# qingstor-incubating/qsfs-fuse

Hardware: AMD Instinct MI355X
Metric: GiB/s MD5-hashed, device-resident 10 MB chunks, batch=512; % HBM-read peak (higher is better)
Workload: dtype u32; 1 GPU; batch=512 x 10 MiB chunks per GPU, device-resident (BASELINE config 2); global_batch=512, chunk_bytes=10485760, parallelism=single GPU, kernel=producer/consumer (qsmd5_batch_pc64_kernel)

## Files before the change

qsfs-fuse_amd/csrc/md5_core.h:

```cpp
#pragma once

#include <hip/hip_runtime.h>
#include <stdint.h>

namespace qsmd5 {

struct Md5Tables {
  static constexpr uint32_t K[64] = {
      0xd76aa478u, 0xe8c7b756u, 0x242070dbu, 0xc1bdceeeu, 0xf57c0fafu, 0x4787c62au,
      0xa8304613u, 0xfd469501u, 0x698098d8u, 0x8b44f7afu, 0xffff5bb1u, 0x895cd7beu,
      0x6b901122u, 0xfd987193u, 0xa679438eu, 0x49b40821u, 0xf61e2562u, 0xc040b340u,
      0x265e5a51u, 0xe9b6c7aau, 0xd62f105du, 0x02441453u, 0xd8a1e681u, 0xe7d3fbc8u,
      0x21e1cde6u, 0xc33707d6u, 0xf4d50d87u, 0x455a14edu, 0xa9e3e905u, 0xfcefa3f8u,
      0x676f02d9u, 0x8d2a4c8au, 0xfffa3942u, 0x8771f681u, 0x6d9d6122u, 0xfde5380cu,
      0xa4beea44u, 0x4bdecfa9u, 0xf6bb4b60u, 0xbebfbc70u, 0x289b7ec6u, 0xeaa127fau,
      0xd4ef3085u, 0x04881d05u, 0xd9d4d039u, 0xe6db99e5u, 0x1fa27cf8u, 0xc4ac5665u,
      0xf4292244u, 0x432aff97u, 0xab9423a7u, 0xfc93a039u, 0x655b59c3u, 0x8f0ccc92u,
      0xffeff47du, 0x85845dd1u, 0x6fa87e4fu, 0xfe2ce6e0u, 0xa3014314u, 0x4e0811a1u,
      0xf7537e82u, 0xbd3af235u, 0x2ad7d2bbu, 0xeb86d391u};
};

constexpr uint32_t kInit0 = 0x67452301u;
constexpr uint32_t kInit1 = 0xefcdab89u;
constexpr uint32_t kInit2 = 0x98badcfeu;
constexpr uint32_t kInit3 = 0x10325476u;

__host__ __device__ constexpr int md5_shift(int i) {
  return (i < 16)   ? ((i & 3) == 0 ? 7 : (i & 3) == 1 ? 12 : (i & 3) == 2 ? 17 : 22)
         : (i < 32) ? ((i & 3) == 0 ? 5 : (i & 3) == 1 ? 9 : (i & 3) == 2 ? 14 : 20)
         : (i < 48) ? ((i & 3) == 0 ? 4 : (i & 3) == 1 ? 11 : (i & 3) == 2 ? 16 : 23)
                    : ((i & 3) == 0 ? 6 : (i & 3) == 1 ? 10 : (i & 3) == 2 ? 15 : 21);
}

__host__ __device__ constexpr int md5_word(int i) {
  return (i < 16) ? i
         : (i < 32) ? ((5 * (i - 16) + 1) & 15)
         : (i < 48) ? ((3 * (i - 32) + 5) & 15)
                    : ((7 * (i - 48)) & 15);
}

__host__ __device__ constexpr uint32_t md5_fn_host(int round, uint32_t x, uint32_t y, uint32_t z) {
  return round == 0   ? ((x & y) | (~x & z))
         : round == 1 ? ((x & z) | (y & ~z))
         : round == 2 ? (x ^ y ^ z)
                      : (y ^ (x | ~z));
}
__host__ __device__ constexpr uint32_t md5_bitop3_imm(int round) {
  return md5_fn_host(round, 0xF0u, 0xCCu, 0xAAu) & 0xFFu;
}

template <int I>
__device__ __forceinline__ uint32_t md5_round_fn(uint32_t b, uint32_t c, uint32_t d) {
  return __builtin_amdgcn_bitop3_b32(b, c, d, md5_bitop3_imm(I >> 4));
}

template <int I>
__device__ __forceinline__ void md5_steps(uint32_t (&v)[4], const uint32_t (&w)[16]) {
  if constexpr (I < 64) {
    constexpr int ia = (4 - (I & 3)) & 3;
    constexpr int ib = (ia + 1) & 3;
    constexpr int ic = (ia + 2) & 3;
    constexpr int id = (ia + 3) & 3;
    const uint32_t amk = v[ia] + w[md5_word(I)] + Md5Tables::K[I];
    const uint32_t t = amk + md5_round_fn<I>(v[ib], v[ic], v[id]);
    v[ia] = v[ib] + __builtin_rotateleft32(t, md5_shift(I));
    md5_steps<I + 1>(v, w);
  }
}

template <int I, int kEnd = 64>
__device__ __forceinline__ void md5_steps_mk(uint32_t (&v)[4], const uint32_t (&mk)[64]) {
  if constexpr (I < kEnd) {
    constexpr int ia = (4 - (I & 3)) & 3;
    constexpr int ib = (ia + 1) & 3;
    constexpr int ic = (ia + 2) & 3;
    constexpr int id = (ia + 3) & 3;
    const uint32_t t = v[ia] + md5_round_fn<I>(v[ib], v[ic], v[id]) + mk[I];
    v[ia] = v[ib] + __builtin_rotateleft32(t, md5_shift(I));
    md5_steps_mk<I + 1, kEnd>(v, mk);
  }
}

__device__ __forceinline__ void md5_compress_mk(uint32_t (&st)[4], const uint32_t (&mk)[64]) {
  uint32_t v[4] = {st[0], st[1], st[2], st[3]};
  md5_steps_mk<0>(v, mk);
  st[0] += v[0];
  st[1] += v[1];
  st[2] += v[2];
  st[3] += v[3];
}

__device__ __forceinline__ void md5_compress(uint32_t (&st)[4], const uint32_t (&w)[16]) {
  uint32_t v[4] = {st[0], st[1], st[2], st[3]};
  md5_steps<0>(v, w);
  st[0] += v[0];
  st[1] += v[1];
  st[2] += v[2];
  st[3] += v[3];
}

typedef uint32_t u32x4 __attribute__((ext_vector_type(4)));
typedef uint32_t u32x4_a4 __attribute__((ext_vector_type(4), aligned(4)));
#define QS_GLOBAL __attribute__((address_space(1)))

template <bool kNT = false>
__device__ __forceinline__ u32x4 load16_a4(const uint32_t* p) {
  if constexpr (kNT)
    return __builtin_nontemporal_load((const QS_GLOBAL u32x4_a4*)(reinterpret_cast<uintptr_t>(p)));
  else
    return *(const QS_GLOBAL u32x4_a4*)(reinterpret_cast<uintptr_t>(p));
}
__device__ __forceinline__ uint32_t load4(const uint32_t* p) {
  return *(const QS_GLOBAL uint32_t*)(reinterpret_cast<uintptr_t>(p));
}

__device__ __forceinline__ void unpack4(uint32_t (&w)[16], int k, u32x4 q) {
  w[4 * k + 0] = q.x;
  w[4 * k + 1] = q.y;
  w[4 * k + 2] = q.z;
  w[4 * k + 3] = q.w;
}

}
```

qsfs-fuse_amd/csrc/md5_kernels.hip:

```cpp
#include <hip/hip_runtime.h>
#include <stdint.h>

#include "md5_core.h"

namespace qsmd5 {

struct ChunkDesc {
  const uint8_t* ptr;
  uint64_t len;
};

__device__ __forceinline__ void blocks_aligned4(uint32_t (&st)[4], const uint32_t* p,
                                                uint32_t nblk) {
  if (nblk == 0) return;
  const uint32_t last = nblk - 1;
  u32x4 a0, a1, a2, a3, b0, b1, b2, b3, c0, c1, c2, c3, d0, d1, d2, d3;
#define QS_LOAD(X, blk)                                   \
  do {                                                    \
    const uint32_t* q_ = p + (uint64_t)(blk) * 16u;       \
    X##0 = load16_a4(q_);                                 \
    X##1 = load16_a4(q_ + 4);                             \
    X##2 = load16_a4(q_ + 8);                             \
    X##3 = load16_a4(q_ + 12);                            \
  } while (0)
#define QS_COMPRESS(X)            \
  do {                            \
    uint32_t w_[16];              \
    unpack4(w_, 0, X##0);         \
    unpack4(w_, 1, X##1);         \
    unpack4(w_, 2, X##2);         \
    unpack4(w_, 3, X##3);         \
    md5_compress(st, w_);         \
  } while (0)
  QS_LOAD(a, 0);
  QS_LOAD(b, min(1u, last));
  QS_LOAD(c, min(2u, last));
  QS_LOAD(d, min(3u, last));
  uint32_t j = 0;
  for (; j + 4 <= nblk; j += 4) {
    QS_COMPRESS(a);
    QS_LOAD(a, min(j + 4, last));
    QS_COMPRESS(b);
    QS_LOAD(b, min(j + 5, last));
    QS_COMPRESS(c);
    QS_LOAD(c, min(j + 6, last));
    QS_COMPRESS(d);
    QS_LOAD(d, min(j + 7, last));
  }
  if (j < nblk) QS_COMPRESS(a);
  if (j + 1 < nblk) QS_COMPRESS(b);
  if (j + 2 < nblk) QS_COMPRESS(c);
#undef QS_COMPRESS
#undef QS_LOAD
}

__device__ __forceinline__ void blocks_unaligned(uint32_t (&st)[4], const uint8_t* bp,
                                                 uint32_t nblk) {
  const uintptr_t a = reinterpret_cast<uintptr_t>(bp);
  const uint32_t* base = reinterpret_cast<const uint32_t*>(a & ~uintptr_t(3));
  const uint32_t off = static_cast<uint32_t>(a & 3u);
  for (uint32_t j = 0; j < nblk; ++j) {
    const uint32_t* q = base + (uint64_t)j * 16u;
    u32x4 x0 = load16_a4(q), x1 = load16_a4(q + 4), x2 = load16_a4(q + 8),
          x3 = load16_a4(q + 12);
    uint32_t e = load4(q + 16);
    uint32_t d[17] = {x0.x, x0.y, x0.z, x0.w, x1.x, x1.y, x1.z, x1.w, x2.x,
                      x2.y, x2.z, x2.w, x3.x, x3.y, x3.z, x3.w, e};
    uint32_t w[16];
#pragma unroll
    for (int k = 0; k < 16; ++k) w[k] = __builtin_amdgcn_alignbyte(d[k + 1], d[k], off);
    md5_compress(st, w);
  }
}

__device__ __forceinline__ void finish(uint32_t (&st)[4], const uint8_t* tp, uint32_t rem,
                                       uint64_t total_len) {
  const uintptr_t a = reinterpret_cast<uintptr_t>(tp);
  const uint32_t* base = reinterpret_cast<const uint32_t*>(a & ~uintptr_t(3));
  const uint32_t off = static_cast<uint32_t>(a & 3u);
  uint32_t d[17];
#pragma unroll
  for (int k = 0; k < 17; ++k)
    d[k] = (rem != 0u && (uint32_t)(4 * k) < off + rem) ? load4(base + k) : 0u;
  uint32_t w[16];
#pragma unroll
  for (int k = 0; k < 16; ++k) {
    uint32_t x = __builtin_amdgcn_alignbyte(d[k + 1], d[k], off);
    const uint32_t lo = 4u * k;
    uint32_t m = rem >= lo + 4u ? 0xffffffffu : rem <= lo ? 0u : ((1u << (8u * (rem - lo))) - 1u);
    x &= m;
    if ((rem >> 2) == (uint32_t)k) x |= 0x80u << (8u * (rem & 3u));
    w[k] = x;
  }
  const uint64_t bits = total_len << 3;
  if (rem < 56u) {
    w[14] = (uint32_t)bits;
    w[15] = (uint32_t)(bits >> 32);
    md5_compress(st, w);
  } else {
    md5_compress(st, w);
#pragma unroll
    for (int k = 0; k < 14; ++k) w[k] = 0u;
    w[14] = (uint32_t)bits;
    w[15] = (uint32_t)(bits >> 32);
    md5_compress(st, w);
  }
}

__device__ __forceinline__ void hash_message(uint32_t (&st)[4], const uint8_t* p, uint64_t len) {
  const uint32_t nblk = (uint32_t)(len >> 6);
  if ((reinterpret_cast<uintptr_t>(p) & 3u) == 0)
    blocks_aligned4(st, reinterpret_cast<const uint32_t*>(p), nblk);
  else
    blocks_unaligned(st, p, nblk);
  finish(st, p + ((uint64_t)nblk << 6), (uint32_t)(len & 63u), len);
}


__device__ __forceinline__ uint32_t wave_max_u32(uint32_t v) {
#pragma unroll
  for (int o = 32; o > 0; o >>= 1) v = max(v, (uint32_t)__shfl_xor((int)v, o, 64));
  return v;
}

__device__ __forceinline__ uint32_t rfl_u32(uint32_t v) {
  return (uint32_t)__builtin_amdgcn_readfirstlane((int)v);
}

__device__ __forceinline__ uint32_t wave_min_u32(uint32_t v) {
#pragma unroll
  for (int o = 32; o > 0; o >>= 1) v = min(v, (uint32_t)__shfl_xor((int)v, o, 64));
  return v;
}

__device__ __forceinline__ void lds_barrier() {
  asm volatile("s_waitcnt lgkmcnt(0)\n\ts_barrier" ::: "memory");
}

constexpr int kPcHalf = 4;
constexpr int kPcLead = 8;
constexpr int kLgkmcnt0 = 0xC07F;

struct PcBlockRegs {
  u32x4 q[4];
  uint32_t e;
};

template <bool kNT>
__device__ __forceinline__ void pc_load_block(PcBlockRegs& r, const uint32_t* base, uint32_t off,
                                              uint32_t blk) {
  const uint32_t* q = base + (uint64_t)blk * 16u;
  r.q[0] = load16_a4<kNT>(q);
  r.q[1] = load16_a4<kNT>(q + 4);
  r.q[2] = load16_a4<kNT>(q + 8);
  r.q[3] = load16_a4<kNT>(q + 12);
  r.e = off ? load4(q + 16) : 0u;
}

__device__ __forceinline__ void pc_write_mk(u32x4 (*slot)[64], uint32_t lane, const PcBlockRegs& r,
                                            uint32_t off) {
  uint32_t d[17] = {r.q[0].x, r.q[0].y, r.q[0].z, r.q[0].w, r.q[1].x, r.q[1].y,
                    r.q[1].z, r.q[1].w, r.q[2].x, r.q[2].y, r.q[2].z, r.q[2].w,
                    r.q[3].x, r.q[3].y, r.q[3].z, r.q[3].w, r.e};
  uint32_t w[16];
#pragma unroll
  for (int k = 0; k < 16; ++k) w[k] = __builtin_amdgcn_alignbyte(d[k + 1], d[k], off);
#pragma unroll
  for (int g = 0; g < 16; ++g) {
    u32x4 m;
    m.x = w[md5_word(4 * g + 0)] + Md5Tables::K[4 * g + 0];
    m.y = w[md5_word(4 * g + 1)] + Md5Tables::K[4 * g + 1];
    m.z = w[md5_word(4 * g + 2)] + Md5Tables::K[4 * g + 2];
    m.w = w[md5_word(4 * g + 3)] + Md5Tables::K[4 * g + 3];
    slot[g][lane] = m;
  }
}


template <bool kAllLive, int kHalf = kPcHalf, int kLead = 0, int kLead2 = 0>
__device__ __forceinline__ void chain_phase(uint32_t (&st)[4], const u32x4 (*ring)[16][64],
                                            uint32_t s0, uint32_t lane, uint32_t blk0,
                                            uint32_t nblk) {
  u32x4 a[16], b[16];
  auto read_slot = [&](u32x4 (&dst)[16], uint32_t slot) {
#pragma unroll
    for (int g = 0; g < 16; ++g) dst[g] = ring[slot][g][lane];
  };
  auto unpack_slot = [&](uint32_t (&mk)[64], const u32x4 (&src)[16]) {
#pragma unroll
    for (int g = 0; g < 16; ++g) {
      mk[4 * g + 0] = src[g].x;
      mk[4 * g + 1] = src[g].y;
      mk[4 * g + 2] = src[g].z;
      mk[4 * g + 3] = src[g].w;
    }
  };
  auto compress_slot = [&](const u32x4 (&src)[16]) {
    uint32_t mk[64];
    unpack_slot(mk, src);
    md5_compress_mk(st, mk);
  };
  read_slot(a, s0);
  if constexpr (kLead > 0) {
    static_assert(kLead % 4 == 0 && kLead < 64, "kLead: whole ds_read_b128 groups");
    __builtin_amdgcn_sched_barrier(0);
    __builtin_amdgcn_s_waitcnt((kLgkmcnt0 & ~(0xF << 8)) | ((16 - kLead / 4) << 8));
    __builtin_amdgcn_sched_barrier(0);
    const bool run0 = kAllLive || blk0 < nblk;
    uint32_t mk[64];
    unpack_slot(mk, a);
    uint32_t v[4] = {st[0], st[1], st[2], st[3]};
    if (run0) md5_steps_mk<0, kLead>(v, mk);
    constexpr int kRest = kLead2 > kLead ? kLead2 : kLead;
    if constexpr (kLead2 > kLead) {
      static_assert(kLead2 % 4 == 0 && kLead2 < 64, "kLead2: whole ds_read_b128 groups");
      __builtin_amdgcn_sched_barrier(0);
      __builtin_amdgcn_s_waitcnt((kLgkmcnt0 & ~(0xF << 8)) | ((16 - kLead2 / 4) << 8));
      __builtin_amdgcn_sched_barrier(0);
      if (run0) md5_steps_mk<kLead, kLead2>(v, mk);
    }
    __builtin_amdgcn_sched_barrier(0);
    __builtin_amdgcn_s_waitcnt(kLgkmcnt0);
    if (1 < kHalf) read_slot(b, s0 + 1);
    __builtin_amdgcn_sched_barrier(0);
    if (run0) {
      md5_steps_mk<kRest, 64>(v, mk);
      st[0] += v[0];
      st[1] += v[1];
      st[2] += v[2];
      st[3] += v[3];
    }
  }
#pragma unroll
  for (int h = (kLead > 0 ? 1 : 0); h < kHalf; ++h) {
    __builtin_amdgcn_sched_barrier(0);
    __builtin_amdgcn_s_waitcnt(kLgkmcnt0);
    if (h + 1 < kHalf) read_slot((h & 1) ? a : b, s0 + h + 1);
    __builtin_amdgcn_sched_barrier(0);
    if (kAllLive || blk0 + (uint32_t)h < nblk) compress_slot((h & 1) ? b : a);
  }
}


}

using namespace qsmd5;

extern "C" __global__ __launch_bounds__(64) void qsmd5_batch_kernel(
    const ChunkDesc* __restrict__ chunks, const uint32_t* __restrict__ order, uint32_t n,
    uint32_t* __restrict__ digests) {
  const uint32_t t = blockIdx.x * 64u + threadIdx.x;
  if (t >= n) return;
  const uint32_t idx = order ? order[t] : t;
  const ChunkDesc cd = chunks[idx];
  uint32_t st[4] = {kInit0, kInit1, kInit2, kInit3};
  hash_message(st, cd.ptr, cd.len);
  u32x4 o = {st[0], st[1], st[2], st[3]};
  *reinterpret_cast<u32x4*>(digests + 4u * (uint64_t)idx) = o;
}

extern "C" __global__ __launch_bounds__(64) void qsmd5_final_kernel(uint32_t* __restrict__ state,
                                                                    const uint8_t* tail,
                                                                    uint32_t rem,
                                                                    uint64_t total_len) {
  if (threadIdx.x != 0 || blockIdx.x != 0) return;
  uint32_t st[4] = {state[0], state[1], state[2], state[3]};
  finish(st, tail, rem, total_len);
  state[0] = st[0];
  state[1] = st[1];
  state[2] = st[2];
  state[3] = st[3];
}

namespace {
constexpr uint32_t kLcgA = 1103515245u;
constexpr uint32_t kLcgC = 12345u;
constexpr uint32_t kSeg = 1024u;

__device__ __forceinline__ uint32_t lcg_jump(uint32_t x, uint64_t n) {
  uint32_t am = kLcgA, cm = kLcgC;
  uint32_t ar = 1u, cr = 0u;
  while (n) {
    if (n & 1u) {
      ar = ar * am;
      cr = cr * am + cm;
    }
    cm = cm * am + cm;
    am = am * am;
    n >>= 1;
  }
  return ar * x + cr;
}
}

extern "C" __global__ __launch_bounds__(256) void qsmd5_lcg_fill_kernel(
    uint8_t* __restrict__ base, uint64_t stride, uint64_t len, uint32_t seed0,
    uint32_t nchunks, uint64_t segs_per_chunk) {
  const uint64_t g = (uint64_t)blockIdx.x * blockDim.x + threadIdx.x;
  const uint64_t chunk = g / segs_per_chunk;
  if (chunk >= nchunks) return;
  const uint64_t seg = g - chunk * segs_per_chunk;
  const uint64_t start = seg * kSeg;
  if (start >= len) return;
  const uint64_t end = start + kSeg < len ? start + kSeg : len;
  uint32_t x = lcg_jump(seed0 + (uint32_t)chunk, start);
  uint8_t* out = base + chunk * stride;
  uint64_t i = start;
  if (((reinterpret_cast<uintptr_t>(out) + start) & 3u) == 0) {
    for (; i + 4 <= end; i += 4) {
      uint32_t v = 0;
#pragma unroll
      for (int b = 0; b < 4; ++b) {
        x = x * kLcgA + kLcgC;
        v |= ((x >> 16) & 0xffu) << (8 * b);
      }
      *reinterpret_cast<uint32_t*>(out + i) = v;
    }
  }
  for (; i < end; ++i) {
    x = x * kLcgA + kLcgC;
    out[i] = (uint8_t)(x >> 16);
  }
}

constexpr uint32_t kSkewMinBlocks = 1u << 19;
template <bool kColumn, int kDepth = 1, int kHalf = kPcHalf, bool kNT = false, bool kTrace = false,
          int kPace = 0, int kGap = 0, int kLead = kPcLead, int kLead2 = 0, int kProbe = 0>
__device__ __forceinline__ void pc_body(const ChunkDesc* __restrict__ chunks,
                                        const uint32_t* __restrict__ order, uint32_t n,
                                        uint32_t* __restrict__ digests, uint64_t col_off,
                                        uint64_t col_w, uint32_t* __restrict__ states,
                                        uint32_t skew, uint64_t* __restrict__ trace = nullptr,
                                        uint32_t lanes = 64) {
  __shared__ u32x4 ring[2 * kHalf][16][64];
  const uint32_t lane = threadIdx.x & 63u;
  const uint32_t wave = threadIdx.x >> 6;
  const uint32_t t = blockIdx.x * lanes + lane;
  const bool live = lane < lanes && t < n;
  uint32_t idx = 0;
  ChunkDesc cd = {nullptr, 0};
  uint64_t seg = 0;
  bool final = true;
  if (live) {
    if (kColumn) {
      idx = order[t];
      cd = chunks[t];
      const uint64_t rest = cd.len - col_off;
      final = rest <= col_w;
      seg = final ? rest : col_w;
    } else {
      idx = order ? order[t] : t;
      cd = chunks[idx];
      seg = cd.len;
    }
  }
  const uint32_t nblk = (uint32_t)(seg >> 6);
  const bool skewed = !kColumn && skew != 0 && wave_max_u32(nblk) >= kSkewMinBlocks;
  const uint32_t delta = (skewed && nblk) ? skew * ((lane * 37u) & 63u) : 0u;
  const uint32_t phases = (wave_max_u32(nblk + delta) + kHalf - 1) / kHalf;
  const uintptr_t pa = reinterpret_cast<uintptr_t>(cd.ptr);
  const uint32_t off = (uint32_t)(pa & 3u);

  if (wave == 1) {
    const uint32_t* base = reinterpret_cast<const uint32_t*>(pa & ~uintptr_t(3));
    const uint32_t last = nblk ? nblk - 1 : 0;
    PcBlockRegs r[kDepth][kHalf];
    if constexpr ((kProbe & 2) != 0) {
#pragma unroll
      for (int k = 0; k < kDepth; ++k)
#pragma unroll
        for (int h = 0; h < kHalf; ++h) r[k][h] = PcBlockRegs{{lane, lane, lane, lane}, lane};
    }
    auto load_phase = [&](PcBlockRegs (&rs)[kHalf], uint32_t p) {
      if constexpr ((kProbe & 2) != 0) return;
      if (nblk) {
#pragma unroll
        for (int h = 0; h < kHalf; ++h) {
          const uint32_t j = p * kHalf + h;
          pc_load_block<kNT>(rs[h], base, off, j < delta ? 0u : min(j - delta, last));
        }
      }
    };
    auto write_phase = [&](const PcBlockRegs (&rs)[kHalf], uint32_t p) {
      if (nblk) {
#pragma unroll
        for (int h = 0; h < kHalf; ++h) {
          if constexpr (kGap > 0) {
            if (h) __builtin_amdgcn_s_sleep(kGap);
          }
          if constexpr ((kProbe & 1) == 0) pc_write_mk(ring[(p & 1u) * kHalf + h], lane, rs[h], off);
        }
      }
    };
    uint64_t t_start = 0, t_wait = 0, t_write = 0;
    if constexpr (kTrace) t_start = __builtin_amdgcn_s_memtime();
    if (phases > 0) {
#pragma unroll
      for (int k = 0; k < kDepth; ++k) load_phase(r[k], (uint32_t)k);
      write_phase(r[0], 0);
      load_phase(r[0], kDepth);
    }
    lds_barrier();
    for (uint32_t p0 = 0; p0 < phases; p0 += kDepth) {
#pragma unroll
      for (int u = 0; u < kDepth; ++u) {
        const uint32_t p = p0 + (uint32_t)u;
        if (p < phases) {
          if (p + 1 < phases) {
            uint64_t tw = 0;
            if constexpr (kTrace) tw = __builtin_amdgcn_s_memtime();
            if constexpr (kPace > 0) __builtin_amdgcn_s_sleep(kPace);
            write_phase(r[(u + 1) % kDepth], p + 1);
            if constexpr (kTrace) t_write += __builtin_amdgcn_s_memtime() - tw;
            load_phase(r[(u + 1) % kDepth], p + 1 + kDepth);
          }
          uint64_t tb = 0;
          if constexpr (kTrace) tb = __builtin_amdgcn_s_memtime();
          lds_barrier();
          if constexpr (kTrace) t_wait += __builtin_amdgcn_s_memtime() - tb;
        }
      }
    }
    if constexpr (kTrace) {
      if (lane == 0) {
        uint64_t* tr = trace + (uint64_t)blockIdx.x * 1024u;
        tr[1019] = __builtin_amdgcn_s_memtime() - t_start;
        tr[1022] = t_wait;
        tr[1023] = t_write;
      }
    }
    return;
  }

  const uint32_t live_lo = rfl_u32((wave_max_u32(delta) + kHalf - 1) / kHalf);
  const uint32_t live_hi = rfl_u32(wave_min_u32(live ? nblk + delta : 0xffffffffu) / kHalf);
  uint32_t st[4] = {kInit0, kInit1, kInit2, kInit3};
  if (kColumn && col_off != 0 && live) {
    const u32x4 s4 = *reinterpret_cast<const u32x4*>(states + 4u * (uint64_t)idx);
    st[0] = s4.x;
    st[1] = s4.y;
    st[2] = s4.z;
    st[3] = s4.w;
  }
  uint64_t c_start = 0, c_wait = 0;
  if constexpr (kTrace) c_start = __builtin_amdgcn_s_memtime();
  lds_barrier();
  for (uint32_t p = 0; p < phases; ++p) {
    if constexpr (kTrace) {
      if (lane == 0 && (p & 4095u) == 0u) {
        uint64_t* tr = trace + (uint64_t)blockIdx.x * 1024u + 2u * (p >> 12);
        tr[0] = __builtin_amdgcn_s_memtime();
        tr[1] = __builtin_amdgcn_s_memrealtime();
      }
    }
    const uint32_t s0 = (p & 1u) * kHalf;
    if (p >= live_lo && p < live_hi)
      chain_phase<true, kHalf, kLead, kLead2>(st, ring, s0, lane, p * kHalf - delta, nblk);
    else
      chain_phase<false, kHalf, kLead, kLead2>(st, ring, s0, lane, p * kHalf - delta, nblk);
    uint64_t tb = 0;
    if constexpr (kTrace) tb = __builtin_amdgcn_s_memtime();
    lds_barrier();
    if constexpr (kTrace) c_wait += __builtin_amdgcn_s_memtime() - tb;
  }
  if constexpr (kTrace) {
    if (lane == 0) {
      uint64_t* tr = trace + (uint64_t)blockIdx.x * 1024u;
      tr[1020] = c_wait;
      tr[1021] = __builtin_amdgcn_s_memtime() - c_start;
    }
  }
  if (!live) return;
  if (kColumn && !final) {
    u32x4 o = {st[0], st[1], st[2], st[3]};
    *reinterpret_cast<u32x4*>(states + 4u * (uint64_t)idx) = o;
    return;
  }
  finish(st, cd.ptr + ((uint64_t)nblk << 6), (uint32_t)(seg & 63u), cd.len);
  u32x4 o = {st[0], st[1], st[2], st[3]};
  *reinterpret_cast<u32x4*>(digests + 4u * (uint64_t)idx) = o;
}

constexpr int kPcDepth = 2;
constexpr int kPcPace = 8;

extern "C" __global__ __launch_bounds__(128) void qsmd5_batch_pc_kernel(
    const ChunkDesc* __restrict__ chunks, const uint32_t* __restrict__ order, uint32_t n,
    uint32_t* __restrict__ digests, uint32_t skew, uint32_t lanes) {
  pc_body<false, kPcDepth, kPcHalf, false, false, kPcPace>(chunks, order, n, digests, 0, ~0ull,
                                                           nullptr, skew, nullptr, lanes);
}

#define QSMD5_PC_FIXED(NAME, LANES, NT)                                                        \
  extern "C" __global__ __launch_bounds__(128) void NAME(                                     \
      const ChunkDesc* __restrict__ chunks, const uint32_t* __restrict__ order, uint32_t n,   \
      uint32_t* __restrict__ digests, uint32_t skew) {                                        \
    pc_body<false, kPcDepth, kPcHalf, NT, false, kPcPace>(chunks, order, n, digests, 0, ~0ull, \
                                                          nullptr, skew, nullptr, LANES);      \
  }
QSMD5_PC_FIXED(qsmd5_batch_pc64_kernel, 64u, false)
QSMD5_PC_FIXED(qsmd5_batch_pc64_nt_kernel, 64u, true)
QSMD5_PC_FIXED(qsmd5_batch_pc32_kernel, 32u, false)
QSMD5_PC_FIXED(qsmd5_batch_pc32_nt_kernel, 32u, true)
#undef QSMD5_PC_FIXED

extern "C" __global__ __launch_bounds__(128) void qsmd5_batch_pc2_kernel(
    const ChunkDesc* __restrict__ chunks, const uint32_t* __restrict__ order, uint32_t n,
    uint32_t* __restrict__ digests, uint32_t skew, uint32_t lanes) {
  pc_body<false, 1, 2>(chunks, order, n, digests, 0, ~0ull, nullptr, skew, nullptr, lanes);
}

extern "C" __global__ __launch_bounds__(128) void qsmd5_batch_pc_nt_kernel(
    const ChunkDesc* __restrict__ chunks, const uint32_t* __restrict__ order, uint32_t n,
    uint32_t* __restrict__ digests, uint32_t skew, uint32_t lanes) {
  pc_body<false, kPcDepth, kPcHalf, true, false, kPcPace>(chunks, order, n, digests, 0, ~0ull,
                                                          nullptr, skew, nullptr, lanes);
}

extern "C" __global__ __launch_bounds__(128) void qsmd5_batch_pc2_nt_kernel(
    const ChunkDesc* __restrict__ chunks, const uint32_t* __restrict__ order, uint32_t n,
    uint32_t* __restrict__ digests, uint32_t skew, uint32_t lanes) {
  pc_body<false, 1, 2, true>(chunks, order, n, digests, 0, ~0ull, nullptr, skew, nullptr, lanes);
}

extern "C" __global__ __launch_bounds__(128) void qsmd5_column_pc_kernel(
    const ChunkDesc* __restrict__ segs, const uint32_t* __restrict__ order, uint32_t n,
    uint32_t* __restrict__ digests, uint64_t col_off, uint64_t col_w,
    uint32_t* __restrict__ states) {
  pc_body<true>(segs, order, n, digests, col_off, col_w, states, 0u);
}

extern "C" __global__ __launch_bounds__(128) void qsmd5_column_pc2_kernel(
    const ChunkDesc* __restrict__ segs, const uint32_t* __restrict__ order, uint32_t n,
    uint32_t* __restrict__ digests, uint64_t col_off, uint64_t col_w,
    uint32_t* __restrict__ states) {
  pc_body<true, 1, 2>(segs, order, n, digests, col_off, col_w, states, 0u);
}

#define QS_GP(p) ((const __attribute__((address_space(1))) void*)(uintptr_t)(p))
#define QS_LP(p) ((__attribute__((address_space(3))) void*)(uintptr_t)(uint32_t)(uintptr_t)(p))

#ifndef QS_COAL_AUX
#define QS_COAL_AUX 2
#endif
template <int U, int kU, int kTB, int kS, int kCPI, bool kImm>
__device__ __forceinline__ void coal_fast_group(uint32_t (&st)[4], const uint8_t* (&gp)[kS],
                                                u32x4 (*tile_buf)[64][kS], uint32_t lane,
                                                uint32_t rswz) {
  if constexpr (U < kU) {
#pragma unroll
    for (int i = 0; i < kS; ++i) {
      if constexpr (kImm) {
        constexpr int kOff = U * kTB * 64;
        __builtin_amdgcn_global_load_lds(
            QS_GP(gp[i]),
            QS_LP(reinterpret_cast<uintptr_t>(&tile_buf[(U + 1) & 1][i * kCPI][0]) - kOff), 16,
            kOff, QS_COAL_AUX);
      } else {
        __builtin_amdgcn_global_load_lds(QS_GP(gp[i]), QS_LP(&tile_buf[(U + 1) & 1][i * kCPI][0]),
                                         16, 0, QS_COAL_AUX);
        gp[i] += kTB * 64;
      }
    }
    asm volatile("s_waitcnt vmcnt(%0)" ::"n"(kS) : "memory");
#pragma unroll
    for (int h = 0; h < kTB; ++h) {
      uint32_t w[16];
      unpack4(w, 0, tile_buf[U & 1][lane][(4 * h + 0) ^ rswz]);
      unpack4(w, 1, tile_buf[U & 1][lane][(4 * h + 1) ^ rswz]);
      unpack4(w, 2, tile_buf[U & 1][lane][(4 * h + 2) ^ rswz]);
      unpack4(w, 3, tile_buf[U & 1][lane][(4 * h + 3) ^ rswz]);
      md5_compress(st, w);
    }
    asm volatile("s_waitcnt lgkmcnt(0)" ::: "memory");
    coal_fast_group<U + 1, kU, kTB, kS, kCPI, kImm>(st, gp, tile_buf, lane, rswz);
  }
}

template <int kTB, int kBufs, bool kImm = false, int kPrioEpoch = 0>
__device__ __forceinline__ void batch_coal_body(const ChunkDesc* __restrict__ chunks,
                                                const uint32_t* __restrict__ order, uint32_t n,
                                                uint32_t* __restrict__ digests) {
  constexpr int kS = 4 * kTB;
  constexpr int kCPI = 64 / kS;
  constexpr int kUImm = 4;
  constexpr int kPad = kImm ? ((kUImm - 1) * kTB * 64 + 15) / 16 : 0;
  __shared__ u32x4 tile_raw[kPad + kBufs * 64 * kS];
  u32x4 (*tile_buf)[64][kS] = reinterpret_cast<u32x4 (*)[64][kS]>(tile_raw + kPad);
  const uint32_t lane = threadIdx.x;
  const uint32_t t = blockIdx.x * 64u + lane;
  uint32_t idx = 0;
  ChunkDesc cd = {nullptr, 0};
  if (t < n) {
    idx = order ? order[t] : t;
    cd = chunks[idx];
  }
  const uint32_t nblk = (uint32_t)(cd.len >> 6);
  const uint32_t ntiles = rfl_u32((wave_max_u32(nblk) + (kTB - 1)) / kTB);
  auto swz = [](uint32_t c) -> uint32_t {
    return kTB == 2 ? ((c >> 1) & 7u) : (c & 15u);
  };

  const uint32_t slot = lane % kS;
  const uint64_t myptr = reinterpret_cast<uint64_t>(cd.ptr);
  const uint8_t* src[kS];
  uint32_t src_nblk[kS], piece[kS];
#pragma unroll
  for (int i = 0; i < kS; ++i) {
    const int c = i * kCPI + (int)(lane / kS);
    const uint32_t lo = (uint32_t)__shfl((int)(uint32_t)myptr, c, 64);
    const uint32_t hi = (uint32_t)__shfl((int)(uint32_t)(myptr >> 32), c, 64);
    src[i] = reinterpret_cast<const uint8_t*>(((uint64_t)hi << 32) | lo);
    src_nblk[i] = (uint32_t)__shfl((int)nblk, c, 64);
    piece[i] = slot ^ swz((uint32_t)c);
  }
  const uint8_t* dummy = reinterpret_cast<const uint8_t*>(chunks);
  auto issue_tile = [&](uint32_t b, uint32_t tl) {
#pragma unroll
    for (int i = 0; i < kS; ++i) {
      const uint32_t blk = min(tl * (uint32_t)kTB + (piece[i] >> 2), src_nblk[i] - 1u);
      const uint8_t* g = src_nblk[i] ? src[i] + (uint64_t)blk * 64u + (piece[i] & 3u) * 16u
                                     : dummy;
      __builtin_amdgcn_global_load_lds(QS_GP(g), QS_LP(&tile_buf[b][i * kCPI][0]), 16, 0,
                                       QS_COAL_AUX);
    }
  };
  const uint32_t rswz = swz(lane);
  uint32_t st[4] = {kInit0, kInit1, kInit2, kInit3};
#pragma unroll
  for (int k = 0; k < kBufs - 1; ++k)
    if ((uint32_t)k < ntiles) issue_tile((uint32_t)k, (uint32_t)k);
  uint32_t tl = 0;
  if constexpr (kBufs == 2) {
    constexpr int kU = kImm ? kUImm : 2;
    const bool full_wave = (blockIdx.x + 1u) * 64u <= n;
    const uint32_t fast_tiles = full_wave ? rfl_u32(wave_min_u32(nblk)) / (uint32_t)kTB : 0u;
    const uint8_t* gp[kS];
#pragma unroll
    for (int i = 0; i < kS; ++i)
      gp[i] = src[i] + kTB * 64u + (piece[i] >> 2) * 64u + (piece[i] & 3u) * 16u;
    for (; tl + (uint32_t)kU < fast_tiles; tl += (uint32_t)kU) {
      if constexpr (kPrioEpoch > 0) {
        const uint32_t wave_id = __builtin_amdgcn_s_getreg((3 << 11) | 4) & 0xfu;
        if (((tl >> kPrioEpoch) ^ wave_id) & 1u) __builtin_amdgcn_s_setprio(1);
        else __builtin_amdgcn_s_setprio(0);
      }
      coal_fast_group<0, kU, kTB, kS, kCPI, kImm>(st, gp, tile_buf, lane, rswz);
      if constexpr (kImm) {
#pragma unroll
        for (int i = 0; i < kS; ++i) gp[i] += kU * kTB * 64;
      }
    }
  }
  for (; tl < ntiles; ++tl) {
    const uint32_t b = tl % kBufs;
    if (tl + (kBufs - 1) < ntiles) {
      issue_tile((tl + (kBufs - 1)) % kBufs, tl + (kBufs - 1));
      if constexpr (kS * (kBufs - 1) == 8) asm volatile("s_waitcnt vmcnt(8)" ::: "memory");
      else if constexpr (kS * (kBufs - 1) == 16) asm volatile("s_waitcnt vmcnt(16)" ::: "memory");
      else asm volatile("s_waitcnt vmcnt(0)" ::: "memory");
    } else {
      asm volatile("s_waitcnt vmcnt(0)" ::: "memory");
    }
#pragma unroll
    for (int h = 0; h < kTB; ++h) {
      u32x4 q0 = tile_buf[b][lane][(4 * h + 0) ^ rswz];
      u32x4 q1 = tile_buf[b][lane][(4 * h + 1) ^ rswz];
      u32x4 q2 = tile_buf[b][lane][(4 * h + 2) ^ rswz];
      u32x4 q3 = tile_buf[b][lane][(4 * h + 3) ^ rswz];
      if (tl * (uint32_t)kTB + h < nblk) {
        uint32_t w[16];
        unpack4(w, 0, q0);
        unpack4(w, 1, q1);
        unpack4(w, 2, q2);
        unpack4(w, 3, q3);
        md5_compress(st, w);
      }
    }
    asm volatile("s_waitcnt lgkmcnt(0)" ::: "memory");
  }
  if (t >= n) return;
  finish(st, cd.ptr + ((uint64_t)nblk << 6), (uint32_t)(cd.len & 63u), cd.len);
  u32x4 o = {st[0], st[1], st[2], st[3]};
  *reinterpret_cast<u32x4*>(digests + 4u * (uint64_t)idx) = o;
}

extern "C" __global__ __launch_bounds__(64) void qsmd5_batch_coal_kernel(
    const ChunkDesc* __restrict__ chunks, const uint32_t* __restrict__ order, uint32_t n,
    uint32_t* __restrict__ digests) {
  batch_coal_body<2, 2>(chunks, order, n, digests);
}

#undef QS_GP
#undef QS_LP

struct GatherRow {
  const uint8_t* src;
  uint8_t* dst;
  uint64_t len;
};

__device__ __forceinline__ void gather_row(const GatherRow g) {
  const uint64_t nvec = g.len >> 4;
  const u32x4* __restrict__ src = reinterpret_cast<const u32x4*>(g.src);
  u32x4* __restrict__ dst = reinterpret_cast<u32x4*>(g.dst);
  constexpr uint32_t kU = 4;
  uint64_t i = threadIdx.x;
  for (; i + (kU - 1) * 256u < nvec; i += kU * 256u) {
    u32x4 v[kU];
#pragma unroll
    for (uint32_t u = 0; u < kU; ++u) v[u] = __builtin_nontemporal_load(src + i + u * 256u);
#pragma unroll
    for (uint32_t u = 0; u < kU; ++u) dst[i + u * 256u] = v[u];
  }
  for (; i < nvec; i += 256u) dst[i] = __builtin_nontemporal_load(src + i);
  const uint64_t tail = g.len & 15u;
  if (threadIdx.x < tail) g.dst[(nvec << 4) + threadIdx.x] = g.src[(nvec << 4) + threadIdx.x];
}

extern "C" __global__ __launch_bounds__(256) void qsmd5_gather_kernel(const GatherRow* __restrict__ rows,
                                                                     uint32_t nrows) {
  for (uint32_t r = blockIdx.x; r < nrows; r += gridDim.x) gather_row(rows[r]);
}

#include "md5_launch.h"

namespace qsmd5 {

static inline void clear_stale_error() { (void)hipGetLastError(); }

hipError_t launch_batch(const void* chunks, const uint32_t* order, uint32_t n, uint32_t* digests,
                        int kind, hipStream_t s, uint32_t skew_blocks, bool load_nt, uint32_t lanes) {
  if (n == 0) return hipSuccess;
  clear_stale_error();
  const uint32_t groups = (n + 63u) / 64u;
  if (lanes < 1 || lanes > 64) return hipErrorInvalidValue;
  const uint32_t pc_groups = (n + lanes - 1) / lanes;
  if (kind == kKernelLatency) {
    const ChunkDesc* c = static_cast<const ChunkDesc*>(chunks);
    const uint32_t skew = skew_blocks / kPcHalf * kPcHalf;
    if (lanes == 64)
      hipLaunchKernelGGL(load_nt ? qsmd5_batch_pc64_nt_kernel : qsmd5_batch_pc64_kernel,
                         dim3(pc_groups), dim3(128), 0, s, c, order, n, digests, skew);
    else if (lanes == 32)
      hipLaunchKernelGGL(load_nt ? qsmd5_batch_pc32_nt_kernel : qsmd5_batch_pc32_kernel,
                         dim3(pc_groups), dim3(128), 0, s, c, order, n, digests, skew);
    else
      hipLaunchKernelGGL(load_nt ? qsmd5_batch_pc_nt_kernel : qsmd5_batch_pc_kernel, dim3(pc_groups),
                         dim3(128), 0, s, c, order, n, digests, skew, lanes);
  } else if (kind == kKernelLatency2) {
    hipLaunchKernelGGL(load_nt ? qsmd5_batch_pc2_nt_kernel : qsmd5_batch_pc2_kernel, dim3(pc_groups),
                       dim3(128), 0, s, static_cast<const ChunkDesc*>(chunks), order, n, digests,
                       skew_blocks / kPcHalf * kPcHalf, lanes);
  } else if (kind == kKernelCoalesced) {
    hipLaunchKernelGGL(qsmd5_batch_coal_kernel, dim3(groups), dim3(64), 0, s,
                       static_cast<const ChunkDesc*>(chunks), order, n, digests);
  } else {
    hipLaunchKernelGGL(qsmd5_batch_kernel, dim3(groups), dim3(64), 0, s,
                       static_cast<const ChunkDesc*>(chunks), order, n, digests);
  }
  return hipGetLastError();
}

hipError_t launch_column(const void* segs, const uint32_t* order, uint32_t n, uint32_t* digests,
                         uint64_t col_off, uint64_t col_w, uint32_t* states, hipStream_t s) {
  if (n == 0) return hipSuccess;
  clear_stale_error();
  if (n > kLatencyKernelResident)
    hipLaunchKernelGGL(qsmd5_column_pc2_kernel, dim3((n + 63u) / 64u), dim3(128), 0, s,
                       static_cast<const ChunkDesc*>(segs), order, n, digests, col_off, col_w,
                       states);
  else
    hipLaunchKernelGGL(qsmd5_column_pc_kernel, dim3((n + 63u) / 64u), dim3(128), 0, s,
                       static_cast<const ChunkDesc*>(segs), order, n, digests, col_off, col_w,
                       states);
  return hipGetLastError();
}


hipError_t launch_gather(const void* rows, uint32_t nrows, hipStream_t s, uint32_t groups) {
  if (nrows == 0) return hipSuccess;
  constexpr size_t kGatherLds = 80u << 10;
  if (groups == 0) groups = 1;
  clear_stale_error();
  hipLaunchKernelGGL(qsmd5_gather_kernel, dim3(nrows < groups ? nrows : groups),
                     dim3(256), kGatherLds, s, static_cast<const GatherRow*>(rows), nrows);
  return hipGetLastError();
}

hipError_t launch_final(uint32_t* state, const uint8_t* tail, uint32_t rem, uint64_t total_len,
                        hipStream_t s) {
  clear_stale_error();
  hipLaunchKernelGGL(qsmd5_final_kernel, dim3(1), dim3(64), 0, s, state, tail, rem, total_len);
  return hipGetLastError();
}

hipError_t warm_up(hipStream_t s) {
  clear_stale_error();
  hipLaunchKernelGGL(qsmd5_lcg_fill_kernel, dim3(1), dim3(64), 0, s, nullptr, 0, 0, 0u, 0u, 1);
  return hipGetLastError();
}

hipError_t launch_lcg_fill(uint8_t* base, uint64_t stride, uint64_t len, uint32_t seed0,
                           uint32_t nchunks, hipStream_t s) {
  if (nchunks == 0 || len == 0) return hipSuccess;
  const uint64_t segs = (len + kSeg - 1) / kSeg;
  const uint64_t threads = segs * nchunks;
  const uint64_t blocks = (threads + 255) / 256;
  if (blocks > 0x7fffffffull) return hipErrorInvalidValue;
  clear_stale_error();
  hipLaunchKernelGGL(qsmd5_lcg_fill_kernel, dim3((uint32_t)blocks), dim3(256), 0, s, base, stride,
                     len, seed0, nchunks, segs);
  return hipGetLastError();
}

}
```

qsfs-fuse_amd/csrc/md5_launch.h:

```cpp
#pragma once

#include <hip/hip_runtime.h>
#include <stdint.h>

namespace qsmd5 {

enum KernelKind : int {
  kKernelThroughput = 0,
  kKernelLatency = 1,
  kKernelCoalesced = 2,
  kKernelLatency2 = 3,
};

constexpr uint32_t kLatencyKernelResident = 256u * 64u;
constexpr uint32_t kLatency2KernelResident = 2u * 256u * 64u;

constexpr uint32_t kPcSkewBlocks = 4;

hipError_t launch_batch(const void* chunks, const uint32_t* order, uint32_t n, uint32_t* digests,
                        int kind, hipStream_t s, uint32_t skew_blocks = kPcSkewBlocks,
                        bool load_nt = false, uint32_t lanes = 64);
hipError_t launch_column(const void* segs, const uint32_t* order, uint32_t n, uint32_t* digests,
                         uint64_t col_off, uint64_t col_w, uint32_t* states, hipStream_t s);
hipError_t launch_final(uint32_t* state, const uint8_t* tail, uint32_t rem, uint64_t total_len,
                        hipStream_t s);
constexpr size_t kGatherRowBytes = 24;
hipError_t launch_gather(const void* rows, uint32_t nrows, hipStream_t s, uint32_t groups);
hipError_t warm_up(hipStream_t s);
hipError_t launch_lcg_fill(uint8_t* base, uint64_t stride, uint64_t len, uint32_t seed0,
                           uint32_t nchunks, hipStream_t s);

}
```

ubench/ubench_md5.hip:

```cpp
#include <hip/hip_runtime.h>
#include <stdint.h>
#include <stdio.h>
#include <stdlib.h>
#include <string.h>

#include <algorithm>
#include <map>
#include <chrono>
#include <vector>

#include "../qsfs-fuse_amd/csrc/md5_kernels.hip"
extern "C" {
#include "../oracle/md5_oracle.c"
}

#define CK(x)                                                                      \
  do {                                                                             \
    hipError_t e_ = (x);                                                           \
    if (e_ != hipSuccess) {                                                        \
      fprintf(stderr, "HIP error %s at %s:%d\n", hipGetErrorString(e_), __FILE__, \
              __LINE__);                                                           \
      exit(2);                                                                     \
    }                                                                              \
  } while (0)

template <int D>
__global__ __launch_bounds__(128) void k_pc_depth(const ChunkDesc* __restrict__ c,
                                                  const uint32_t* __restrict__ o, uint32_t n,
                                                  uint32_t* __restrict__ d, uint32_t skew) {
  pc_body<false, D>(c, o, n, d, 0, ~0ull, nullptr, skew);
}

__global__ __launch_bounds__(128) void k_pc_half2(const ChunkDesc* __restrict__ c,
                                                  const uint32_t* __restrict__ o, uint32_t n,
                                                  uint32_t* __restrict__ d, uint32_t skew) {
  pc_body<false, 1, 2>(c, o, n, d, 0, ~0ull, nullptr, skew);
}

__global__ __launch_bounds__(128) void k_pc_trace(const ChunkDesc* __restrict__ c,
                                                  const uint32_t* __restrict__ o, uint32_t n,
                                                  uint32_t* __restrict__ d, uint32_t skew,
                                                  uint64_t* __restrict__ tr, uint32_t lanes) {
  pc_body<false, kPcDepth, kPcHalf, false, true, kPcPace>(c, o, n, d, 0, ~0ull, nullptr, skew, tr,
                                                          lanes);
}

template <int kProbe>
__global__ __launch_bounds__(128) void k_pc_probe(const ChunkDesc* __restrict__ c,
                                                  const uint32_t* __restrict__ o, uint32_t n,
                                                  uint32_t* __restrict__ d, uint32_t skew) {
  pc_body<false, kPcDepth, kPcHalf, false, false, kPcPace, 0, kPcLead, 0, kProbe>(
      c, o, n, d, 0, ~0ull, nullptr, skew, nullptr, 64u);
}

template <int kR, int kHalf = kPcHalf>
__device__ __forceinline__ void chain_phase_spread(uint32_t (&st)[4], const u32x4 (*ring)[16][64],
                                                   uint32_t s0, uint32_t lane) {
  u32x4 a[16], b[16];
#pragma unroll
  for (int g = 0; g < 16; ++g) a[g] = ring[s0][g][lane];
#pragma unroll
  for (int h = 0; h < kHalf; ++h) {
    __builtin_amdgcn_sched_barrier(0);
    __builtin_amdgcn_s_waitcnt(kLgkmcnt0);
    __builtin_amdgcn_sched_barrier(0);
    u32x4 (&cur)[16] = (h & 1) ? b : a;
    u32x4 (&nxt)[16] = (h & 1) ? a : b;
    if (h + 1 < kHalf) {
#pragma unroll
      for (int g = 0; g < 16; ++g) nxt[g] = ring[s0 + h + 1][g][lane];
    }
    uint32_t mk[64];
#pragma unroll
    for (int g = 0; g < 16; ++g) {
      mk[4 * g + 0] = cur[g].x;
      mk[4 * g + 1] = cur[g].y;
      mk[4 * g + 2] = cur[g].z;
      mk[4 * g + 3] = cur[g].w;
    }
    md5_compress_mk(st, mk);
    if (h + 1 < kHalf) {
#pragma unroll
      for (int g = 0; g < 16; ++g) {
        __builtin_amdgcn_sched_group_barrier(0x0100, 1, 0);
        __builtin_amdgcn_sched_group_barrier(0x0002, kR, 0);
      }
    }
  }
}

template <int kR>
__global__ __launch_bounds__(128) void k_chain_spread(uint64_t* out, uint32_t* sink, int phases) {
  __shared__ u32x4 ring[2 * kPcHalf][16][64];
  const uint32_t lane = threadIdx.x & 63u, wave = threadIdx.x >> 6;
  for (int k = threadIdx.x; k < 2 * kPcHalf * 16 * 64; k += blockDim.x)
    (&ring[0][0][0])[k] = u32x4{(uint32_t)k * 2654435761u, (uint32_t)k, 7u, 9u};
  __syncthreads();
  if (wave == 1) return;
  uint32_t st[4] = {kInit0, kInit1, kInit2, kInit3};
  const uint64_t t0 = __builtin_amdgcn_s_memtime();
  for (int p = 0; p < phases; ++p) chain_phase_spread<kR>(st, ring, (uint32_t)(p & 1) * kPcHalf, lane);
  const uint64_t t1 = __builtin_amdgcn_s_memtime();
  if (lane == 0) out[0] = t1 - t0;
  sink[lane] = st[0] ^ st[1] ^ st[2] ^ st[3];
}

template <int kMode, uint32_t kLanes = 64, int kL = 0>
__global__ __launch_bounds__(128) void k_chain_cost(uint64_t* out, uint32_t* sink, int phases) {
  __shared__ u32x4 ring[2 * kPcHalf][16][64];
  const uint32_t lane = threadIdx.x & 63u, wave = threadIdx.x >> 6;
  for (int k = threadIdx.x; k < 2 * kPcHalf * 16 * 64; k += blockDim.x)
    (&ring[0][0][0])[k] = u32x4{(uint32_t)k * 2654435761u, (uint32_t)k, 7u, 9u};
  __syncthreads();
  if (wave == 1) {
    if (kMode == 1)
      for (int p = 0; p < phases; ++p) lds_barrier();
    return;
  }
  if (lane >= kLanes) return;
  uint32_t st[4] = {kInit0, kInit1, kInit2, kInit3};
  uint32_t mk[64];
#pragma unroll
  for (int i = 0; i < 64; ++i) mk[i] = (&ring[0][0][0])[i * 64 + lane].x;
  const uint64_t t0 = __builtin_amdgcn_s_memtime();
  for (int p = 0; p < phases; ++p) {
    if constexpr (kMode == 2) {
#pragma unroll
      for (int h = 0; h < kPcHalf; ++h) md5_compress_mk(st, mk);
      asm volatile("" : "+v"(st[0]), "+v"(st[1]));
    } else {
      chain_phase<true, kPcHalf, kL>(st, ring, (uint32_t)(p & 1) * kPcHalf, lane, 0, 1u << 30);
      if (kMode == 1) lds_barrier();
    }
  }
  const uint64_t t1 = __builtin_amdgcn_s_memtime();
  if (lane == 0) out[0] = t1 - t0;
  sink[lane] = st[0] ^ st[1] ^ st[2] ^ st[3];
}

template <int kSrc, int kRing = 8>
__global__ __launch_bounds__(128) void k_chain_ring(uint64_t* out, uint32_t* sink, int blocks,
                                                    const u32x4* __restrict__ gring) {
  __shared__ u32x4 ring[8][16][64];
  const uint32_t lane = threadIdx.x & 63u, wave = threadIdx.x >> 6;
  if (kSrc == 0) {
    for (int k = threadIdx.x; k < 8 * 16 * 64; k += blockDim.x)
      (&ring[0][0][0])[k] = u32x4{(uint32_t)k * 2654435761u, (uint32_t)k, 7u, 9u};
    __syncthreads();
  }
  if (wave == 1) return;
  constexpr int kAux = kSrc == 1 ? 0 : kSrc == 2 ? 1 : 2;
  const auto rs = __builtin_amdgcn_make_buffer_rsrc((void*)gring, 0, kRing * 16384, 0x00020000);
  u32x4 a[16], b[16];
  auto read_blk = [&](u32x4 (&dst)[16], uint32_t blk) {
    const uint32_t slot = blk & (kRing - 1);
#pragma unroll
    for (int g = 0; g < 16; ++g) {
      if constexpr (kSrc == 0)
        dst[g] = ring[blk & 7u][g][lane];
      else
        dst[g] = __builtin_bit_cast(
            u32x4, __builtin_amdgcn_raw_buffer_load_b128(rs, (int)(lane * 16u + g * 1024u),
                                                         (int)(slot * 16384u), kAux));
    }
  };
  auto compress = [&](uint32_t (&st)[4], const u32x4 (&src)[16]) {
    uint32_t mk[64];
#pragma unroll
    for (int g = 0; g < 16; ++g) {
      mk[4 * g + 0] = src[g].x;
      mk[4 * g + 1] = src[g].y;
      mk[4 * g + 2] = src[g].z;
      mk[4 * g + 3] = src[g].w;
    }
    md5_compress_mk(st, mk);
  };
  constexpr int kWait = kSrc == 0 ? kLgkmcnt0 : 0x0F70;
  uint32_t st[4] = {kInit0, kInit1, kInit2, kInit3};
  read_blk(a, 0);
  const uint64_t t0 = __builtin_amdgcn_s_memtime();
  for (int h = 0; h < blocks; h += 2) {
    __builtin_amdgcn_sched_barrier(0);
    __builtin_amdgcn_s_waitcnt(kWait);
    read_blk(b, h + 1);
    __builtin_amdgcn_sched_barrier(0);
    compress(st, a);
    __builtin_amdgcn_sched_barrier(0);
    __builtin_amdgcn_s_waitcnt(kWait);
    read_blk(a, h + 2);
    __builtin_amdgcn_sched_barrier(0);
    compress(st, b);
  }
  const uint64_t t1 = __builtin_amdgcn_s_memtime();
  if (lane == 0) out[0] = t1 - t0;
  sink[lane] = st[0] ^ st[1] ^ st[2] ^ st[3];
}

template <int kS>
__global__ __launch_bounds__(128) void k_chain_at(uint64_t* out, uint32_t* sink, int blocks,
                                                  const u32x4* __restrict__ gring) {
  (void)gring;
  __shared__ u32x4 ring[8][16][64];
  const uint32_t lane = threadIdx.x & 63u, wave = threadIdx.x >> 6;
  for (int k = threadIdx.x; k < 8 * 16 * 64; k += blockDim.x)
    (&ring[0][0][0])[k] = u32x4{(uint32_t)k * 2654435761u, (uint32_t)k, 7u, 9u};
  __syncthreads();
  if (wave == 1) return;
  u32x4 a[16], b[16];
  auto read_blk = [&](u32x4 (&dst)[16], uint32_t blk) {
#pragma unroll
    for (int g = 0; g < 16; ++g) dst[g] = ring[blk & 7u][g][lane];
  };
  uint32_t st[4] = {kInit0, kInit1, kInit2, kInit3};
  auto block = [&](const u32x4 (&cur)[16], u32x4 (&nxt)[16], uint32_t next_blk) {
    uint32_t mk[64];
#pragma unroll
    for (int g = 0; g < 16; ++g) {
      mk[4 * g + 0] = cur[g].x;
      mk[4 * g + 1] = cur[g].y;
      mk[4 * g + 2] = cur[g].z;
      mk[4 * g + 3] = cur[g].w;
    }
    __builtin_amdgcn_sched_barrier(0);
    __builtin_amdgcn_s_waitcnt(kLgkmcnt0);
    __builtin_amdgcn_sched_barrier(0);
    uint32_t v[4] = {st[0], st[1], st[2], st[3]};
    if constexpr (kS > 0) md5_steps_mk<0, kS>(v, mk);
    __builtin_amdgcn_sched_barrier(0);
    read_blk(nxt, next_blk);
    __builtin_amdgcn_sched_barrier(0);
    md5_steps_mk<kS, 64>(v, mk);
    st[0] += v[0];
    st[1] += v[1];
    st[2] += v[2];
    st[3] += v[3];
  };
  read_blk(a, 0);
  const uint64_t t0 = __builtin_amdgcn_s_memtime();
  for (int h = 0; h < blocks; h += 2) {
    block(a, b, h + 1);
    block(b, a, h + 2);
  }
  const uint64_t t1 = __builtin_amdgcn_s_memtime();
  if (lane == 0) out[0] = t1 - t0;
  sink[lane] = st[0] ^ st[1] ^ st[2] ^ st[3];
}

template <int kSlots, int kLanes, bool kBar, bool kCompact = true>
__global__ __launch_bounds__(128) void k_chain_l1(uint64_t* out, uint32_t* sink, int blocks,
                                                  const u32x4* __restrict__ gring) {
  const uint32_t lane = threadIdx.x & 63u, wave = threadIdx.x >> 6;
  if (wave == 1) {
    if (kBar)
      for (int p = 0; p < blocks + 1; ++p) __builtin_amdgcn_s_barrier();
    return;
  }
  constexpr uint32_t kRow = kCompact ? kLanes * 16u : 1024u;
  constexpr uint32_t kSlotB = 16u * kRow;
  const auto rs = __builtin_amdgcn_make_buffer_rsrc((void*)gring, 0, kSlots * kSlotB, 0x00020000);
  const uint32_t vbase = lane < (uint32_t)kLanes ? lane * 16u : 0x40000000u;
  u32x4 a[16], b[16];
  auto read_blk = [&](u32x4 (&dst)[16], uint32_t slot) {
#pragma unroll
    for (int g = 0; g < 16; ++g)
      dst[g] = __builtin_bit_cast(
          u32x4, __builtin_amdgcn_raw_buffer_load_b128(rs, (int)(vbase + g * kRow),
                                                       (int)(slot * kSlotB), 0));
  };
  auto compress = [&](uint32_t (&st)[4], const u32x4 (&src)[16]) {
    uint32_t mk[64];
#pragma unroll
    for (int g = 0; g < 16; ++g) {
      mk[4 * g + 0] = src[g].x;
      mk[4 * g + 1] = src[g].y;
      mk[4 * g + 2] = src[g].z;
      mk[4 * g + 3] = src[g].w;
    }
    md5_compress_mk(st, mk);
  };
  uint32_t st[4] = {kInit0, kInit1, kInit2, kInit3};
  uint32_t slot = 0;
  auto next = [&]() { slot = slot + 1 == (uint32_t)kSlots ? 0u : slot + 1; return slot; };
  read_blk(a, 0);
  const uint64_t t0 = __builtin_amdgcn_s_memtime();
  for (int h = 0; h < blocks; h += 2) {
    __builtin_amdgcn_sched_barrier(0);
    __builtin_amdgcn_s_waitcnt(0x0F70);
    read_blk(b, next());
    __builtin_amdgcn_sched_barrier(0);
    compress(st, a);
    if (kBar) __builtin_amdgcn_s_barrier();
    __builtin_amdgcn_sched_barrier(0);
    __builtin_amdgcn_s_waitcnt(0x0F70);
    read_blk(a, next());
    __builtin_amdgcn_sched_barrier(0);
    compress(st, b);
    if (kBar) __builtin_amdgcn_s_barrier();
  }
  const uint64_t t1 = __builtin_amdgcn_s_memtime();
  if (kBar) __builtin_amdgcn_s_barrier();
  if (lane == 0) out[0] = t1 - t0;
  sink[lane] = st[0] ^ st[1] ^ st[2] ^ st[3];
}

template <int kStoreAux>
__global__ __launch_bounds__(128) void k_l1_handoff(uint64_t* out, uint32_t* sink, int blocks,
                                                    u32x4* __restrict__ gring) {
  const uint32_t lane = threadIdx.x & 63u, wave = threadIdx.x >> 6;
  const auto rs = __builtin_amdgcn_make_buffer_rsrc((void*)gring, 0, 2 * 16384, 0x00020000);
  if (wave == 1) {
    auto put = [&](uint32_t blk) {
#pragma unroll
      for (int g = 0; g < 16; ++g)
        __builtin_amdgcn_raw_buffer_store_b128(
            __builtin_bit_cast(__attribute__((ext_vector_type(4))) int,
                               u32x4{blk, lane, (uint32_t)g, 0x5au}),
            rs, (int)(lane * 16u + g * 1024u), (int)((blk & 1u) * 16384u), kStoreAux);
    };
    put(0);
    put(1);
    __builtin_amdgcn_s_waitcnt(0x0F70);
    __builtin_amdgcn_s_barrier();
    for (int h = 0; h < blocks; ++h) {
      put((uint32_t)h + 2u);
      __builtin_amdgcn_s_waitcnt(0x0F70);
      __builtin_amdgcn_s_barrier();
    }
    return;
  }
  u32x4 a[16], b[16];
  auto read_blk = [&](u32x4 (&dst)[16], uint32_t blk) {
#pragma unroll
    for (int g = 0; g < 16; ++g)
      dst[g] = __builtin_bit_cast(
          u32x4, __builtin_amdgcn_raw_buffer_load_b128(rs, (int)(lane * 16u + g * 1024u),
                                                       (int)((blk & 1u) * 16384u), 0));
  };
  uint32_t bad = 0;
  auto compress = [&](uint32_t (&st)[4], const u32x4 (&src)[16], uint32_t blk) {
    uint32_t mk[64];
#pragma unroll
    for (int g = 0; g < 16; ++g) {
      bad += (src[g].x != blk) | (src[g].y != lane) | (src[g].z != (uint32_t)g);
      mk[4 * g + 0] = src[g].x;
      mk[4 * g + 1] = src[g].y;
      mk[4 * g + 2] = src[g].z;
      mk[4 * g + 3] = src[g].w;
    }
    md5_compress_mk(st, mk);
  };
  uint32_t st[4] = {kInit0, kInit1, kInit2, kInit3};
  __builtin_amdgcn_s_barrier();
  read_blk(a, 0);
  __builtin_amdgcn_s_waitcnt(0x0F70);
  const uint64_t t0 = __builtin_amdgcn_s_memtime();
  for (int h = 0; h < blocks; h += 2) {
    __builtin_amdgcn_sched_barrier(0);
    read_blk(b, (uint32_t)h + 1u);
    __builtin_amdgcn_sched_barrier(0);
    compress(st, a, (uint32_t)h);
    __builtin_amdgcn_sched_barrier(0);
    __builtin_amdgcn_s_waitcnt(0x0F70);
    __builtin_amdgcn_s_barrier();
    __builtin_amdgcn_sched_barrier(0);
    read_blk(a, (uint32_t)h + 2u);
    __builtin_amdgcn_sched_barrier(0);
    compress(st, b, (uint32_t)h + 1u);
    __builtin_amdgcn_sched_barrier(0);
    __builtin_amdgcn_s_waitcnt(0x0F70);
    __builtin_amdgcn_s_barrier();
  }
  const uint64_t t1 = __builtin_amdgcn_s_memtime();
  if (lane == 0) out[0] = t1 - t0;
  bad = __builtin_amdgcn_readfirstlane(bad) + 0u;
  if (lane == 0) out[1] = bad;
  sink[lane] = st[0] ^ st[1] ^ st[2] ^ st[3];
}

template <int kP, int kG = 0, int kD = 1>
__global__ __launch_bounds__(128) void k_pc_pace(const ChunkDesc* __restrict__ c,
                                                 const uint32_t* __restrict__ o, uint32_t n,
                                                 uint32_t* __restrict__ d, uint32_t skew) {
  pc_body<false, kD, kPcHalf, false, false, kP, kG>(c, o, n, d, 0, ~0ull, nullptr, skew);
}

template <int kL, int kL2 = 0, int kP = 8, int kD = 2>
__global__ __launch_bounds__(128) void k_pc_lead(const ChunkDesc* __restrict__ c,
                                                 const uint32_t* __restrict__ o, uint32_t n,
                                                 uint32_t* __restrict__ d, uint32_t skew) {
  pc_body<false, kD, kPcHalf, false, false, kP, 0, kL, kL2>(c, o, n, d, 0, ~0ull, nullptr, skew, nullptr,
                                                      64u);
}

template <int kP, int kD>
__global__ __launch_bounds__(128) void k_pc2_pace(const ChunkDesc* __restrict__ c,
                                                  const uint32_t* __restrict__ o, uint32_t n,
                                                  uint32_t* __restrict__ d, uint32_t skew) {
  pc_body<false, kD, 2, false, false, kP>(c, o, n, d, 0, ~0ull, nullptr, skew, nullptr, 64u);
}

__global__ __launch_bounds__(128) void k_pc_half5(const ChunkDesc* __restrict__ c,
                                                  const uint32_t* __restrict__ o, uint32_t n,
                                                  uint32_t* __restrict__ d, uint32_t skew) {
  pc_body<false, 1, 5>(c, o, n, d, 0, ~0ull, nullptr, skew);
}

__global__ __launch_bounds__(64) void k_coal_imm(const ChunkDesc* __restrict__ c,
                                                 const uint32_t* __restrict__ o, uint32_t n,
                                                 uint32_t* __restrict__ d) {
  batch_coal_body<2, 2, true>(c, o, n, d);
}

#define REP8(x) x x x x x x x x
#define REP64(x) REP8(REP8(x))

__global__ void k_dep_add(uint64_t* out, uint32_t* sink, int iters) {
  uint32_t v0 = threadIdx.x, v1 = 3;
  uint64_t t0 = __builtin_amdgcn_s_memtime();
  for (int i = 0; i < iters; ++i) {
    asm volatile(REP64("v_add_u32 %0, %0, %1\n") : "+v"(v0) : "v"(v1));
  }
  uint64_t t1 = __builtin_amdgcn_s_memtime();
  if (threadIdx.x == 0) out[0] = t1 - t0;
  sink[threadIdx.x] = v0;
}

__global__ void k_ind_add(uint64_t* out, uint32_t* sink, int iters) {
  uint32_t a = threadIdx.x, b = a + 1, c = a + 2, d = a + 3, one = 1;
  uint64_t t0 = __builtin_amdgcn_s_memtime();
  for (int i = 0; i < iters; ++i) {
    asm volatile(REP8(REP8("v_add_u32 %0, %0, %4\nv_add_u32 %1, %1, %4\nv_add_u32 %2, %2, %4\nv_add_u32 %3, %3, %4\n"))
                 : "+v"(a), "+v"(b), "+v"(c), "+v"(d)
                 : "v"(one));
  }
  uint64_t t1 = __builtin_amdgcn_s_memtime();
  if (threadIdx.x == 0) out[0] = t1 - t0;
  sink[threadIdx.x] = a + b + c + d;
}

__global__ void k_dep_alignbit(uint64_t* out, uint32_t* sink, int iters) {
  uint32_t v0 = threadIdx.x;
  uint64_t t0 = __builtin_amdgcn_s_memtime();
  for (int i = 0; i < iters; ++i) {
    asm volatile(REP64("v_alignbit_b32 %0, %0, %0, 7\n") : "+v"(v0));
  }
  uint64_t t1 = __builtin_amdgcn_s_memtime();
  if (threadIdx.x == 0) out[0] = t1 - t0;
  sink[threadIdx.x] = v0;
}

__global__ void k_dep_bitop3(uint64_t* out, uint32_t* sink, int iters) {
  uint32_t v0 = threadIdx.x, v1 = 5, v2 = 9;
  uint64_t t0 = __builtin_amdgcn_s_memtime();
  for (int i = 0; i < iters; ++i) {
    asm volatile(REP64("v_bitop3_b32 %0, %0, %1, %2 bitop3:0xca\n") : "+v"(v0) : "v"(v1), "v"(v2));
  }
  uint64_t t1 = __builtin_amdgcn_s_memtime();
  if (threadIdx.x == 0) out[0] = t1 - t0;
  sink[threadIdx.x] = v0;
}

__global__ void k_dep_add3(uint64_t* out, uint32_t* sink, int iters) {
  uint32_t v0 = threadIdx.x, v1 = 5, v2 = 9;
  uint64_t t0 = __builtin_amdgcn_s_memtime();
  for (int i = 0; i < iters; ++i) {
    asm volatile(REP64("v_add3_u32 %0, %0, %1, %2\n") : "+v"(v0) : "v"(v1), "v"(v2));
  }
  uint64_t t1 = __builtin_amdgcn_s_memtime();
  if (threadIdx.x == 0) out[0] = t1 - t0;
  sink[threadIdx.x] = v0;
}

__global__ void k_md5_step(uint64_t* out, uint32_t* sink, int iters) {
  uint32_t a = threadIdx.x, b = 1, c = 2, d = 3, m = 7, t = 0, s;
  asm volatile("s_mov_b32 %0, 0x12345" : "=s"(s));
  uint64_t t0 = __builtin_amdgcn_s_memtime();
  for (int i = 0; i < iters; ++i) {
    asm volatile(REP8(REP8(
        "v_add3_u32 %4, %0, %5, %6\n"
        "v_bitop3_b32 %0, %1, %2, %3 bitop3:0xca\n"
        "v_add_u32 %0, %0, %4\n"
        "v_alignbit_b32 %0, %0, %0, 25\n"
        "v_add_u32 %0, %0, %1\n"))
                 : "+v"(a), "+v"(b), "+v"(c), "+v"(d), "+v"(t)
                 : "v"(m), "s"(s));
  }
  uint64_t t1 = __builtin_amdgcn_s_memtime();
  if (threadIdx.x == 0) out[0] = t1 - t0;
  sink[threadIdx.x] = a + b + c + d;
}

__global__ void k_md5_step4(uint64_t* out, uint32_t* sink, int iters) {
  uint32_t a = threadIdx.x, b = 1, c = 2, d = 3, mk = 7;
  uint64_t t0 = __builtin_amdgcn_s_memtime();
  for (int i = 0; i < iters; ++i) {
    asm volatile(REP8(REP8(
        "v_bitop3_b32 %0, %1, %2, %3 bitop3:0xca\n"
        "v_add3_u32 %0, %0, %4, %1\n"
        "v_alignbit_b32 %0, %0, %0, 25\n"
        "v_add_u32 %0, %0, %1\n"))
                 : "+v"(a), "+v"(b), "+v"(c), "+v"(d)
                 : "v"(mk));
  }
  uint64_t t1 = __builtin_amdgcn_s_memtime();
  if (threadIdx.x == 0) out[0] = t1 - t0;
  sink[threadIdx.x] = a + b + c + d;
}

__global__ void k_mix_lds(uint64_t* out, uint32_t* sink, int iters) {
  __shared__ u32x4 lds[64];
  lds[threadIdx.x] = u32x4{threadIdx.x, 1, 2, 3};
  __syncthreads();
  uint32_t v0 = threadIdx.x, v1 = 3;
  u32x4 r;
  uint32_t addr = threadIdx.x * 16;
  uint64_t t0 = __builtin_amdgcn_s_memtime();
  for (int i = 0; i < iters; ++i) {
    asm volatile(REP64("ds_read_b128 %2, %3\n v_add_u32 %0, %0, %1\n v_add_u32 %0, %0, %1\n v_add_u32 %0, %0, %1\n v_add_u32 %0, %0, %1\n")
                 : "+v"(v0), "+v"(v1), "=&v"(r) : "v"(addr));
    asm volatile("s_waitcnt lgkmcnt(0)" ::: "memory");
  }
  uint64_t t1 = __builtin_amdgcn_s_memtime();
  if (threadIdx.x == 0) out[0] = t1 - t0;
  sink[threadIdx.x] = v0 + r.x;
}

typedef void (*ukern)(uint64_t*, uint32_t*, int);

static double run_issue(ukern k, int instr_per_iter, int iters, int threads) {
  uint64_t* d_out;
  uint32_t* d_sink;
  CK(hipMalloc(&d_out, 8));
  CK(hipMalloc(&d_sink, 4 * 1024));
  hipLaunchKernelGGL(k, dim3(1), dim3(threads), 0, 0, d_out, d_sink, 10);
  CK(hipDeviceSynchronize());
  hipLaunchKernelGGL(k, dim3(1), dim3(threads), 0, 0, d_out, d_sink, iters);
  CK(hipDeviceSynchronize());
  uint64_t cyc;
  CK(hipMemcpy(&cyc, d_out, 8, hipMemcpyDeviceToHost));
  CK(hipFree(d_out));
  CK(hipFree(d_sink));
  return (double)cyc / ((double)iters * instr_per_iter);
}

template <int kPrioEpoch>
__global__ __launch_bounds__(64) void k_coal_stamped(const ChunkDesc* __restrict__ chunks, uint32_t n,
                                                     uint32_t* __restrict__ digests, uint64_t* stamps) {
  extern __shared__ uint32_t pad_lds[];
  const uint64_t c0 = __builtin_amdgcn_s_memtime();
  const uint64_t r0 = __builtin_amdgcn_s_memrealtime();
  batch_coal_body<2, 2, false, kPrioEpoch>(chunks, nullptr, n, digests);
  const uint64_t c1 = __builtin_amdgcn_s_memtime();
  const uint64_t r1 = __builtin_amdgcn_s_memrealtime();
  const uint32_t hw = __builtin_amdgcn_s_getreg((31 << 11) | 4);
  const uint32_t xcc = __builtin_amdgcn_s_getreg((31 << 11) | 20);
  if (threadIdx.x == 0) {
    uint64_t* q = stamps + 6ull * blockIdx.x;
    q[0] = c0;
    q[1] = r0;
    q[2] = c1;
    q[3] = r1;
    q[4] = hw;
    q[5] = xcc | ((uint64_t)pad_lds[0] << 63 >> 63 << 32);
  }
}

static double pctl(std::vector<double> v, double q) {
  std::sort(v.begin(), v.end());
  return v[(size_t)std::min<double>(v.size() - 1, q * (v.size() - 1) + 0.5)];
}

static void run_stamps(uint32_t n, uint64_t L, int reps, uint64_t pad, uint32_t extra_lds, int prio = 0) {
  const uint64_t stride = L + pad;
  uint8_t* d_data;
  CK(hipMalloc(&d_data, stride * (uint64_t)n));
  const uint64_t segs = (L + 1023) / 1024, thr = segs * (uint64_t)n;
  hipLaunchKernelGGL(qsmd5_lcg_fill_kernel, dim3((thr + 255) / 256), dim3(256), 0, 0, d_data, stride, L,
                     12345u, n, segs);
  std::vector<ChunkDesc> h(n);
  for (uint32_t i = 0; i < n; ++i) h[i] = {d_data + stride * (uint64_t)i, L};
  ChunkDesc* d_desc;
  uint32_t* d_dig;
  uint64_t* d_st;
  const uint32_t waves = (n + 63) / 64;
  CK(hipMalloc(&d_desc, sizeof(ChunkDesc) * n));
  CK(hipMalloc(&d_dig, 16ull * n));
  CK(hipMalloc(&d_st, 48ull * waves));
  CK(hipMemcpy(d_desc, h.data(), sizeof(ChunkDesc) * n, hipMemcpyHostToDevice));
  hipEvent_t e0, e1;
  CK(hipEventCreate(&e0));
  CK(hipEventCreate(&e1));
  std::vector<uint64_t> st(6ull * waves);
  for (int rep = 0; rep <= reps; ++rep) {
    CK(hipEventRecord(e0, 0));
    if (prio == 0)
      hipLaunchKernelGGL(k_coal_stamped<0>, dim3(waves), dim3(64), extra_lds, 0, d_desc, n, d_dig, d_st);
    else if (prio == 2)
      hipLaunchKernelGGL(k_coal_stamped<2>, dim3(waves), dim3(64), extra_lds, 0, d_desc, n, d_dig, d_st);
    else
      hipLaunchKernelGGL(k_coal_stamped<4>, dim3(waves), dim3(64), extra_lds, 0, d_desc, n, d_dig, d_st);
    CK(hipEventRecord(e1, 0));
    CK(hipEventSynchronize(e1));
    float ms = 0;
    CK(hipEventElapsedTime(&ms, e0, e1));
    CK(hipMemcpy(st.data(), d_st, st.size() * 8, hipMemcpyDeviceToHost));
    if (rep == 0) continue;
    uint64_t r_min = ~0ull, r_max = 0;
    for (uint32_t w = 0; w < waves; ++w) {
      r_min = std::min(r_min, st[6 * w + 1]);
      r_max = std::max(r_max, st[6 * w + 3]);
    }
    auto cu_key = [&](uint32_t w) {
      const uint64_t hw = st[6 * w + 4], xcc = st[6 * w + 5] & 0xf;
      return (xcc << 16) | ((hw >> 8) & 0xff);
    };
    auto simd_key = [&](uint32_t w) { return (cu_key(w) << 2) | ((st[6 * w + 4] >> 4) & 3); };
    std::map<uint64_t, int> per_cu, per_simd;
    for (uint32_t w = 0; w < waves; ++w) {
      ++per_cu[cu_key(w)];
      ++per_simd[simd_key(w)];
    }
    std::vector<double> clk(waves), start_us(waves), end_us(waves);
    double alive = 0;
    std::map<int, std::pair<double, int>> life_by_simd_load;
    for (uint32_t w = 0; w < waves; ++w) {
      const double dr = (double)(st[6 * w + 3] - st[6 * w + 1]);
      clk[w] = dr > 0 ? (double)(st[6 * w + 2] - st[6 * w + 0]) / (dr * 10.0) : 0.0;
      start_us[w] = (st[6 * w + 1] - r_min) * 0.01;
      end_us[w] = (st[6 * w + 3] - r_min) * 0.01;
      alive += dr * 0.01;
      auto& e = life_by_simd_load[per_simd[simd_key(w)]];
      e.first += dr * 0.01;
      e.second += 1;
    }
    std::map<int, int> cu_hist, simd_hist;
    for (auto& kv : per_cu) ++cu_hist[kv.second];
    for (auto& kv : per_simd) ++simd_hist[kv.second];
    const double span_us = (r_max - r_min) * 0.01;
    printf("{\"mode\": \"stamps\", \"prio_epoch\": %d, \"chains\": %u, \"chunk_KiB\": %llu, \"extra_lds\": %u, \"rep\": %d, "
           "\"event_ms\": %.4f, \"GBps\": %.1f, \"span_us\": %.1f, \"clock_GHz_p10_p50_p90\": [%.3f, %.3f, %.3f], "
           "\"start_us_p50_max\": [%.1f, %.1f], \"end_us_min_p50_max\": [%.1f, %.1f, %.1f], "
           "\"alive_share\": %.4f, \"cus\": %zu, \"simds\": %zu",
           prio, n, (unsigned long long)(L >> 10), extra_lds, rep, ms, (double)n * L / (ms * 1e-3) / 1e9, span_us,
           pctl(clk, 0.1), pctl(clk, 0.5), pctl(clk, 0.9), pctl(start_us, 0.5), pctl(start_us, 1.0),
           pctl(end_us, 0.0), pctl(end_us, 0.5), pctl(end_us, 1.0), alive / (waves * span_us), per_cu.size(),
           per_simd.size());
    printf(", \"waves_per_cu_hist\": {");
    bool first = true;
    for (auto& kv : cu_hist) printf("%s\"%d\": %d", first ? "" : ", ", kv.first, kv.second), first = false;
    printf("}, \"waves_per_simd_hist\": {");
    first = true;
    for (auto& kv : simd_hist) printf("%s\"%d\": %d", first ? "" : ", ", kv.first, kv.second), first = false;
    printf("}, \"mean_life_us_by_waves_on_simd\": {");
    first = true;
    for (auto& kv : life_by_simd_load)
      printf("%s\"%d\": %.1f", first ? "" : ", ", kv.first, kv.second.first / kv.second.second), first = false;
    printf("}}\n");
    fflush(stdout);
  }
  int bad = 0;
  std::vector<uint8_t> buf(L);
  uint8_t got[16], want[16];
  for (uint32_t k = 0; k < 64; ++k) {
    const uint32_t i = (uint32_t)(((uint64_t)k * 2039u) % n);
    CK(hipMemcpy(buf.data(), d_data + stride * (uint64_t)i, L, hipMemcpyDeviceToHost));
    CK(hipMemcpy(got, d_dig + 4ull * i, 16, hipMemcpyDeviceToHost));
    oracle_md5(buf.data(), L, want);
    bad += memcmp(got, want, 16) != 0;
  }
  printf("{\"mode\": \"stamps_parity\", \"prio_epoch\": %d, \"chunk_KiB\": %llu, \"checked\": 64, \"bad\": %d}\n",
         prio, (unsigned long long)(L >> 10), bad);
  CK(hipEventDestroy(e0));
  CK(hipEventDestroy(e1));
  CK(hipFree(d_st));
  CK(hipFree(d_dig));
  CK(hipFree(d_desc));
  CK(hipFree(d_data));
}

static bool g_host_pinned = false;
static uint32_t g_skew = kPcSkewBlocks;

static int g_interleave = 0;
static void run_md5(int B, uint64_t L, int reps, bool check, int which = 0, uint64_t pad = 0) {
  uint64_t stride = ((L + 255) & ~uint64_t(255)) + pad;
  uint8_t* d_data;
  if (g_host_pinned)
    CK(hipHostMalloc(&d_data, stride * (uint64_t)B, hipHostMallocDefault));
  else
    CK(hipMalloc(&d_data, stride * (uint64_t)B));
  const uint64_t segs = (L + 1023) / 1024;
  const uint64_t thr = segs * (uint64_t)B;
  hipLaunchKernelGGL(qsmd5_lcg_fill_kernel, dim3((thr + 255) / 256), dim3(256), 0, 0, d_data,
                     stride, L, 12345u, (uint32_t)B, segs);
  std::vector<ChunkDesc> h(B);
  for (int i = 0; i < B; ++i) {
    h[i].ptr = d_data + stride * (uint64_t)i;
    h[i].len = L;
  }
  if (g_interleave) {
    std::vector<ChunkDesc> p(h);
    uint64_t x = 88172645463325252ull;
    auto rnd = [&]() { x ^= x << 13; x ^= x >> 7; x ^= x << 17; return x; };
    if (g_interleave == 1 && B % 64 == 0)
      for (int i = 0; i < B; ++i) p[i] = h[(uint64_t)(i % 64) * (B / 64) + i / 64];
    const int grp = g_interleave == 2 ? 64 : B;
    if (g_interleave >= 2)
      for (int g0 = 0; g0 < B; g0 += grp)
        for (int i = std::min(B, g0 + grp) - 1; i > g0; --i) std::swap(p[i], p[g0 + rnd() % (i - g0 + 1)]);
    h = p;
  }
  ChunkDesc* d_desc;
  uint32_t* d_dig;
  CK(hipMalloc(&d_desc, sizeof(ChunkDesc) * B));
  CK(hipMalloc(&d_dig, 16 * (size_t)B));
  CK(hipMemcpy(d_desc, h.data(), sizeof(ChunkDesc) * B, hipMemcpyHostToDevice));
  hipEvent_t e0, e1;
  CK(hipEventCreate(&e0));
  CK(hipEventCreate(&e1));
  const int grid = (B + 63) / 64;
  auto launch = [&]() {
    if (which == 0)
      hipLaunchKernelGGL(qsmd5_batch_kernel, dim3(grid), dim3(64), 0, 0, d_desc, nullptr,
                         (uint32_t)B, d_dig);
    else if (which == 1)
      hipLaunchKernelGGL(qsmd5_batch_pc64_kernel, dim3(grid), dim3(128), 0, 0, d_desc, nullptr,
                         (uint32_t)B, d_dig, g_skew);
    else if (which == 19)
      hipLaunchKernelGGL(qsmd5_batch_pc_kernel, dim3(grid), dim3(128), 0, 0, d_desc, nullptr,
                         (uint32_t)B, d_dig, g_skew, 64u);
    else if (which == 2)
      hipLaunchKernelGGL(qsmd5_batch_coal_kernel, dim3(grid), dim3(64), 0, 0, d_desc, nullptr,
                         (uint32_t)B, d_dig);
    else if (which == 3)
      hipLaunchKernelGGL(k_pc_depth<2>, dim3(grid), dim3(128), 0, 0, d_desc, nullptr, (uint32_t)B,
                         d_dig, g_skew);
    else if (which == 5)
      hipLaunchKernelGGL(k_pc_half2, dim3(grid), dim3(128), 0, 0, d_desc, nullptr, (uint32_t)B,
                         d_dig, g_skew);
    else if (which == 6)
      hipLaunchKernelGGL(k_coal_imm, dim3(grid), dim3(64), 0, 0, d_desc, nullptr, (uint32_t)B,
                         d_dig);
    else if (which == 7)
      hipLaunchKernelGGL(k_pc_half5, dim3(grid), dim3(128), 0, 0, d_desc, nullptr, (uint32_t)B,
                         d_dig, 0u);
    else if (which == 20)
      hipLaunchKernelGGL((k_pc_pace<0,0,1>), dim3(grid), dim3(128), 0, 0, d_desc, nullptr, (uint32_t)B,
                         d_dig, g_skew);
    else if (which == 21)
      hipLaunchKernelGGL((k_pc_pace<8,0,1>), dim3(grid), dim3(128), 0, 0, d_desc, nullptr, (uint32_t)B,
                         d_dig, g_skew);
    else if (which == 22)
      hipLaunchKernelGGL((k_pc_pace<10,0,1>), dim3(grid), dim3(128), 0, 0, d_desc, nullptr, (uint32_t)B,
                         d_dig, g_skew);
    else if (which == 23)
      hipLaunchKernelGGL((k_pc_pace<8,0,2>), dim3(grid), dim3(128), 0, 0, d_desc, nullptr, (uint32_t)B,
                         d_dig, g_skew);
    else if (which == 24)
      hipLaunchKernelGGL((k_pc_pace<16,0,2>), dim3(grid), dim3(128), 0, 0, d_desc, nullptr, (uint32_t)B,
                         d_dig, g_skew);
    else if (which == 25)
      hipLaunchKernelGGL((k_pc_pace<24,0,2>), dim3(grid), dim3(128), 0, 0, d_desc, nullptr, (uint32_t)B,
                         d_dig, g_skew);
    else if (which == 26)
      hipLaunchKernelGGL((k_pc_pace<32,0,2>), dim3(grid), dim3(128), 0, 0, d_desc, nullptr, (uint32_t)B,
                         d_dig, g_skew);
    else if (which == 30)
      hipLaunchKernelGGL(k_pc_lead<8>, dim3(grid), dim3(128), 0, 0, d_desc, nullptr, (uint32_t)B,
                         d_dig, g_skew);
    else if (which == 31)
      hipLaunchKernelGGL((k_pc_lead<8, 24>), dim3(grid), dim3(128), 0, 0, d_desc, nullptr, (uint32_t)B,
                         d_dig, g_skew);
    else if (which == 32)
      hipLaunchKernelGGL((k_pc_lead<4, 16>), dim3(grid), dim3(128), 0, 0, d_desc, nullptr, (uint32_t)B,
                         d_dig, g_skew);
    else if (which == 35)
      hipLaunchKernelGGL((k_pc_lead<8, 0, 4, 2>), dim3(grid), dim3(128), 0, 0, d_desc, nullptr,
                         (uint32_t)B, d_dig, g_skew);
    else if (which == 36)
      hipLaunchKernelGGL((k_pc_lead<8, 0, 12, 2>), dim3(grid), dim3(128), 0, 0, d_desc, nullptr,
                         (uint32_t)B, d_dig, g_skew);
    else if (which == 37)
      hipLaunchKernelGGL((k_pc_lead<8, 0, 8, 3>), dim3(grid), dim3(128), 0, 0, d_desc, nullptr,
                         (uint32_t)B, d_dig, g_skew);
    else if (which == 38)
      hipLaunchKernelGGL((k_pc_lead<8, 0, 16, 3>), dim3(grid), dim3(128), 0, 0, d_desc, nullptr,
                         (uint32_t)B, d_dig, g_skew);
    else if (which == 39)
      hipLaunchKernelGGL((k_pc_lead<8, 0, 0, 2>), dim3(grid), dim3(128), 0, 0, d_desc, nullptr,
                         (uint32_t)B, d_dig, g_skew);
    else if (which == 40)
      hipLaunchKernelGGL((k_pc2_pace<0, 1>), dim3(grid), dim3(128), 0, 0, d_desc, nullptr,
                         (uint32_t)B, d_dig, g_skew);
    else if (which == 41)
      hipLaunchKernelGGL((k_pc2_pace<0, 2>), dim3(grid), dim3(128), 0, 0, d_desc, nullptr,
                         (uint32_t)B, d_dig, g_skew);
    else if (which == 42)
      hipLaunchKernelGGL((k_pc2_pace<4, 2>), dim3(grid), dim3(128), 0, 0, d_desc, nullptr,
                         (uint32_t)B, d_dig, g_skew);
    else if (which == 43)
      hipLaunchKernelGGL((k_pc2_pace<8, 2>), dim3(grid), dim3(128), 0, 0, d_desc, nullptr,
                         (uint32_t)B, d_dig, g_skew);
    else if (which == 44)
      hipLaunchKernelGGL((k_pc2_pace<2, 2>), dim3(grid), dim3(128), 0, 0, d_desc, nullptr,
                         (uint32_t)B, d_dig, g_skew);
    else if (which == 34)
      hipLaunchKernelGGL((k_pc_lead<0>), dim3(grid), dim3(128), 0, 0, d_desc, nullptr, (uint32_t)B,
                         d_dig, g_skew);
    else if (which == 33)
      hipLaunchKernelGGL((k_pc_lead<8, 32>), dim3(grid), dim3(128), 0, 0, d_desc, nullptr, (uint32_t)B,
                         d_dig, g_skew);
    else if (which == 50)
      hipLaunchKernelGGL(k_pc_probe<1>, dim3(grid), dim3(128), 0, 0, d_desc, nullptr, (uint32_t)B,
                         d_dig, g_skew);
    else if (which == 51)
      hipLaunchKernelGGL(k_pc_probe<2>, dim3(grid), dim3(128), 0, 0, d_desc, nullptr, (uint32_t)B,
                         d_dig, g_skew);
    else if (which == 52)
      hipLaunchKernelGGL(k_pc_probe<3>, dim3(grid), dim3(128), 0, 0, d_desc, nullptr, (uint32_t)B,
                         d_dig, g_skew);
    else
      hipLaunchKernelGGL(k_pc_depth<3>, dim3(grid), dim3(128), 0, 0, d_desc, nullptr, (uint32_t)B,
                         d_dig, g_skew);
  };
  launch();
  CK(hipGetLastError());
  CK(hipDeviceSynchronize());
  std::vector<float> ms(reps);
  for (int r = 0; r < reps; ++r) {
    CK(hipEventRecord(e0, 0));
    launch();
    CK(hipEventRecord(e1, 0));
    CK(hipEventSynchronize(e1));
    CK(hipEventElapsedTime(&ms[r], e0, e1));
  }
  float best = ms[0], med;
  for (float m : ms) best = m < best ? m : best;
  std::vector<float> s = ms;
  std::sort(s.begin(), s.end());
  med = s[s.size() / 2];
  double gib = (double)L * B / (1u << 30);
  if (pad) printf("(stride pad %llu) ", (unsigned long long)pad);
  if ((which == 1 || which == 3 || which == 4 || which == 5) && g_skew)
    printf("(skew %u) ", g_skew);
  if (g_host_pinned) printf("[pinned host, zero-copy] ");
  printf("md5[%s] B=%d L=%llu: median %.3f ms best %.3f ms -> %.2f GiB/s total, r1=%.4f GiB/s/chain, "
         "%.1f cycles/block @2.4GHz\n",
         which == 0 ? "v1" : which == 1 ? "pc" : which == 2 ? "coal" : which == 3 ? "pc-d2" : which == 5 ? "pc-h2" : which == 6 ? "coal-imm" : which == 19 ? "pc (runtime lanes)" : which == 20 ? "pc-r1 (depth 1, no pause)" : which == 21 ? "pace8" : which == 22 ? "pace10" : which == 23 ? "d2-pace8" : which == 24 ? "d2-pace16" : which == 25 ? "d2-pace24" : which == 26 ? "d2-pace32" : which == 30 ? "lead8" : which == 31 ? "lead8+24" : which == 32 ? "lead4+16" : which == 33 ? "lead8+32" : which == 34 ? "lead0 (no graded wait)" : which == 40 ? "pc2 d1 (64u fixed)" : which == 41 ? "pc2 d2" : which == 42 ? "pc2 d2 pace4" : which == 43 ? "pc2 d2 pace8" : which == 44 ? "pc2 d2 pace2" : which == 35 ? "lead8 pace4" : which == 36 ? "lead8 pace12" : which == 37 ? "lead8 pace8 depth3" : which == 38 ? "lead8 pace16 depth3" : which == 39 ? "lead8 no pause" : which == 50 ? "probe: producer writes no ring" : which == 51 ? "probe: producer loads nothing" : which == 52 ? "probe: producer neither loads nor writes" : "pc-d3", B, (unsigned long long)L, med, best, gib / (med / 1e3), (double)L / (1u << 30) / (med / 1e3),
         (med / 1e3) * 2.4e9 / (double)(L / 64));
  if (check) {
    std::vector<uint32_t> dig(4 * (size_t)B);
    CK(hipMemcpy(dig.data(), d_dig, 16 * (size_t)B, hipMemcpyDeviceToHost));
    std::vector<uint8_t> host(L);
    int bad = 0;
    int ncheck = B < 16 ? B : 16;
    for (int i = 0; i < ncheck; ++i) {
      int ci = (i * 7919) % B;
      CK(hipMemcpy(host.data(), d_data + stride * (uint64_t)ci, L, hipMemcpyDeviceToHost));
      std::vector<uint8_t> ref(L);
      oracle_lcg_fill(ref.data(), L, 12345u + ci);
      if (memcmp(ref.data(), host.data(), L) != 0) {
        printf("  generator mismatch chunk %d\n", ci);
        ++bad;
      }
      uint8_t od[16];
      oracle_md5(host.data(), L, od);
      if (memcmp(od, &dig[4 * (size_t)ci], 16) != 0) {
        char hx[33], hg[33];
        oracle_md5_hex(od, hx);
        oracle_md5_hex((const uint8_t*)&dig[4 * (size_t)ci], hg);
        printf("  DIGEST MISMATCH chunk %d: oracle %s gpu %s\n", ci, hx, hg);
        ++bad;
      }
    }
    printf("  check %d chunks: %s\n", ncheck, bad ? "FAIL" : "ok");
  }
  if (g_host_pinned) CK(hipHostFree(d_data)); else CK(hipFree(d_data));
  CK(hipFree(d_desc));
  CK(hipFree(d_dig));
}

static int run_edges(int which) {
  const uint64_t lens[] = {0, 1, 3, 55, 56, 57, 63, 64, 65, 119, 120, 127, 128, 1000, 4096, 8191, 100003};
  const int nl = sizeof(lens) / sizeof(lens[0]);
  int bad = 0;
  uint8_t* d;
  CK(hipMalloc(&d, 1 << 20));
  std::vector<uint8_t> h(1 << 20);
  oracle_lcg_fill(h.data(), h.size(), 777u);
  CK(hipMemcpy(d, h.data(), h.size(), hipMemcpyHostToDevice));
  std::vector<ChunkDesc> desc;
  std::vector<std::pair<uint64_t, uint64_t>> ref;
  for (int off = 0; off < 8; ++off)
    for (int i = 0; i < nl; ++i) {
      uint64_t o = which >= 2 ? off * 4096 + 16 * off : off * 4099 + off;
      desc.push_back({d + o, lens[i]});
      ref.push_back({o, lens[i]});
    }
  int n = desc.size();
  ChunkDesc* dd;
  uint32_t* dg;
  CK(hipMalloc(&dd, sizeof(ChunkDesc) * n));
  CK(hipMalloc(&dg, 16 * n));
  CK(hipMemcpy(dd, desc.data(), sizeof(ChunkDesc) * n, hipMemcpyHostToDevice));
  CK(hipMemset(dg, 0, 16 * n));
  if (which == 0)
    hipLaunchKernelGGL(qsmd5_batch_kernel, dim3((n + 63) / 64), dim3(64), 0, 0, dd, nullptr,
                       (uint32_t)n, dg);
  else if (which == 1)
    hipLaunchKernelGGL(qsmd5_batch_pc64_kernel, dim3((n + 63) / 64), dim3(128), 0, 0, dd, nullptr,
                       (uint32_t)n, dg, g_skew);
  else if (which == 19)
    hipLaunchKernelGGL(qsmd5_batch_pc_kernel, dim3((n + 63) / 64), dim3(128), 0, 0, dd, nullptr,
                       (uint32_t)n, dg, g_skew, 64u);
  else if (which == 2)
    hipLaunchKernelGGL(qsmd5_batch_coal_kernel, dim3((n + 63) / 64), dim3(64), 0, 0, dd, nullptr,
                       (uint32_t)n, dg);
  else if (which == 3)
    hipLaunchKernelGGL(k_pc_depth<2>, dim3((n + 63) / 64), dim3(128), 0, 0, dd, nullptr,
                       (uint32_t)n, dg, g_skew);
  else if (which == 5)
    hipLaunchKernelGGL(k_pc_half2, dim3((n + 63) / 64), dim3(128), 0, 0, dd, nullptr,
                       (uint32_t)n, dg, g_skew);
  else if (which == 6)
    hipLaunchKernelGGL(k_coal_imm, dim3((n + 63) / 64), dim3(64), 0, 0, dd, nullptr, (uint32_t)n,
                       dg);
  else if (which == 7)
    hipLaunchKernelGGL(k_pc_half5, dim3((n + 63) / 64), dim3(128), 0, 0, dd, nullptr, (uint32_t)n,
                       dg, 0u);
  else if (which == 21)
    hipLaunchKernelGGL((k_pc_pace<8, 0, 1>), dim3((n + 63) / 64), dim3(128), 0, 0, dd, nullptr,
                       (uint32_t)n, dg, g_skew);
  else if (which == 24)
    hipLaunchKernelGGL((k_pc_pace<16, 0, 2>), dim3((n + 63) / 64), dim3(128), 0, 0, dd, nullptr,
                       (uint32_t)n, dg, g_skew);
  else if (which >= 30 && which <= 33) {
    auto k = which == 30 ? k_pc_lead<8> : which == 31 ? k_pc_lead<8, 24>
           : which == 32 ? k_pc_lead<4, 16> : k_pc_lead<8, 32>;
    hipLaunchKernelGGL(k, dim3((n + 63) / 64), dim3(128), 0, 0, dd, nullptr, (uint32_t)n, dg, g_skew);
  } else
    hipLaunchKernelGGL(k_pc_depth<3>, dim3((n + 63) / 64), dim3(128), 0, 0, dd, nullptr,
                       (uint32_t)n, dg, g_skew);
  CK(hipDeviceSynchronize());
  std::vector<uint8_t> got(16 * n);
  CK(hipMemcpy(got.data(), dg, 16 * n, hipMemcpyDeviceToHost));
  for (int i = 0; i < n; ++i) {
    uint8_t od[16];
    oracle_md5(h.data() + ref[i].first, ref[i].second, od);
    if (memcmp(od, &got[16 * i], 16)) {
      printf("  edge mismatch off=%llu len=%llu\n", (unsigned long long)ref[i].first,
             (unsigned long long)ref[i].second);
      ++bad;
    }
  }
  printf("edges[%d]: %d cases, %d bad\n", which, n, bad);
  CK(hipFree(d));
  CK(hipFree(dd));
  CK(hipFree(dg));
  return bad;
}

__global__ __launch_bounds__(256) void k_stream_read(const u32x4* __restrict__ p, uint64_t n16,
                                                     uint32_t* sink) {
  u32x4 acc = {0, 0, 0, 0};
  for (uint64_t i = (uint64_t)blockIdx.x * 256 + threadIdx.x; i < n16;
       i += (uint64_t)gridDim.x * 256) {
    u32x4 v = __builtin_nontemporal_load(p + i);
    acc ^= v;
  }
  if ((acc.x ^ acc.y ^ acc.z ^ acc.w) == 0x12345678u) sink[0] = 1;
}

template <bool kNT>
__global__ __launch_bounds__(64) void k_lane_stream(const uint8_t* __restrict__ base,
                                                    uint64_t stride, uint32_t nblk,
                                                    uint32_t* sink) {
  const uint32_t t = blockIdx.x * 64 + threadIdx.x;
  const u32x4* p = reinterpret_cast<const u32x4*>(base + stride * t);
  u32x4 acc = {0, 0, 0, 0};
  for (uint32_t j = 0; j < nblk; j += 8) {
    u32x4 v[32];
#pragma unroll
    for (int k = 0; k < 32; ++k) v[k] = kNT ? __builtin_nontemporal_load(p + 4 * j + k) : p[4 * j + k];
#pragma unroll
    for (int k = 0; k < 32; ++k) acc ^= v[k];
  }
  if ((acc.x ^ acc.y ^ acc.z ^ acc.w) == 0x12345678u) sink[0] = t;
}

static void run_lane_stream(uint32_t B, uint64_t L, uint64_t pad, bool nt) {
  uint64_t stride = L + pad;
  uint8_t* d;
  uint32_t* sink;
  CK(hipMalloc(&d, stride * B));
  CK(hipMalloc(&sink, 4));
  CK(hipMemset(d, 3, stride * B));
  hipEvent_t e0, e1;
  CK(hipEventCreate(&e0));
  CK(hipEventCreate(&e1));
  float best = 1e30f;
  for (int r = 0; r < 4; ++r) {
    CK(hipEventRecord(e0, 0));
    if (nt)
      hipLaunchKernelGGL(k_lane_stream<true>, dim3(B / 64), dim3(64), 0, 0, d, stride,
                         (uint32_t)(L / 64), sink);
    else
      hipLaunchKernelGGL(k_lane_stream<false>, dim3(B / 64), dim3(64), 0, 0, d, stride,
                         (uint32_t)(L / 64), sink);
    CK(hipEventRecord(e1, 0));
    CK(hipEventSynchronize(e1));
    float ms;
    CK(hipEventElapsedTime(&ms, e0, e1));
    if (r) best = ms < best ? ms : best;
  }
  printf("lane_stream%s B=%u L=%llu pad=%llu: %.3f ms -> %.1f GB/s\n", nt ? "[nt]" : "", B,
         (unsigned long long)L, (unsigned long long)pad, best, (double)L * B / (best * 1e-3) / 1e9);
  CK(hipFree(d));
  CK(hipFree(sink));
}

static void run_stream_read(uint64_t bytes, int reps) {
  u32x4* d;
  uint32_t* sink;
  CK(hipMalloc(&d, bytes));
  CK(hipMalloc(&sink, 4));
  CK(hipMemset(d, 1, bytes));
  hipEvent_t e0, e1;
  CK(hipEventCreate(&e0));
  CK(hipEventCreate(&e1));
  float best = 1e30f;
  for (int r = 0; r < reps; ++r) {
    CK(hipEventRecord(e0, 0));
    hipLaunchKernelGGL(k_stream_read, dim3(256 * 8), dim3(256), 0, 0, d, bytes / 16, sink);
    CK(hipEventRecord(e1, 0));
    CK(hipEventSynchronize(e1));
    float ms;
    CK(hipEventElapsedTime(&ms, e0, e1));
    best = ms < best ? ms : best;
  }
  printf("stream_read %llu bytes: best %.3f ms -> %.1f GB/s\n", (unsigned long long)bytes, best,
         bytes / (best * 1e-3) / 1e9);
  CK(hipFree(d));
  CK(hipFree(sink));
}

static void run_h2d(size_t total, size_t piece, int nstreams) {
  void* h = nullptr;
  void* d = nullptr;
  CK(hipHostMalloc(&h, total, hipHostMallocDefault));
  CK(hipMalloc(&d, total));
  memset(h, 1, total);
  hipStream_t st[4];
  for (int i = 0; i < nstreams; ++i) CK(hipStreamCreateWithFlags(&st[i], hipStreamNonBlocking));
  double best = 1e30;
  for (int r = 0; r < 3; ++r) {
    CK(hipDeviceSynchronize());
    auto t0 = std::chrono::steady_clock::now();
    int k = 0;
    for (size_t o = 0; o < total; o += piece, ++k)
      CK(hipMemcpyAsync((char*)d + o, (char*)h + o, std::min(piece, total - o),
                        hipMemcpyHostToDevice, st[k % nstreams]));
    CK(hipDeviceSynchronize());
    double s = std::chrono::duration<double>(std::chrono::steady_clock::now() - t0).count();
    best = std::min(best, s);
  }
  printf("h2d total=%.1f GiB piece=%.0f MiB streams=%d: %.3f s -> %.2f GiB/s (%.1f GB/s)\n",
         total / 1073741824.0, piece / 1048576.0, nstreams, best, total / 1073741824.0 / best,
         total / 1e9 / best);
  for (int i = 0; i < nstreams; ++i) CK(hipStreamDestroy(st[i]));
  CK(hipFree(d));
  CK(hipHostFree(h));
}

static void run_h2d_2d(int rows, size_t len, size_t width, int nstreams) {
  const size_t skew = 4352;
  const size_t total = (size_t)rows * len;
  void* h = nullptr;
  void* d = nullptr;
  CK(hipHostMalloc(&h, total, hipHostMallocDefault));
  CK(hipMalloc(&d, (size_t)rows * (len + skew)));
  memset(h, 1, total);
  hipStream_t st[4];
  for (int i = 0; i < nstreams; ++i) CK(hipStreamCreateWithFlags(&st[i], hipStreamNonBlocking));
  double best = 1e30;
  for (int r = 0; r < 3; ++r) {
    CK(hipDeviceSynchronize());
    auto t0 = std::chrono::steady_clock::now();
    int k = 0;
    for (size_t o = 0; o < len; o += width, ++k)
      CK(hipMemcpy2DAsync((char*)d + o, len + skew, (char*)h + o, len, std::min(width, len - o),
                          rows, hipMemcpyHostToDevice, st[k % nstreams]));
    CK(hipDeviceSynchronize());
    double s = std::chrono::duration<double>(std::chrono::steady_clock::now() - t0).count();
    best = std::min(best, s);
  }
  std::vector<uint8_t> probe(16);
  CK(hipMemcpy(probe.data(), (char*)d + (size_t)(rows - 1) * (len + skew) + len - 16, 16,
               hipMemcpyDeviceToHost));
  printf("h2d-2d rows=%d len=%.1f MiB width=%.2f MiB streams=%d: %.3f s -> %.2f GiB/s (%.1f GB/s)%s\n",
         rows, len / 1048576.0, width / 1048576.0, nstreams, best, total / 1073741824.0 / best,
         total / 1e9 / best, probe[15] == 1 ? "" : "  PLACEMENT WRONG");
  for (int i = 0; i < nstreams; ++i) CK(hipStreamDestroy(st[i]));
  CK(hipFree(d));
  CK(hipHostFree(h));
}


#define QS_GP(p) ((const __attribute__((address_space(1))) void*)(uintptr_t)(p))
#define QS_LP(p) ((__attribute__((address_space(3))) void*)(uintptr_t)(uint32_t)(uintptr_t)(p))
template <int kMode>
__global__ __launch_bounds__(64) void k_coal_probe(const ChunkDesc* __restrict__ chunks, uint32_t n,
                                                   uint32_t* __restrict__ digests,
                                                   uint64_t* __restrict__ stamps) {
  constexpr int kTB = 2, kBufs = 2, kS = 8, kCPI = 8;
  __shared__ u32x4 tile_buf[kBufs][64][kS];
  const uint64_t m0 = __builtin_amdgcn_s_memtime(), r0 = __builtin_amdgcn_s_memrealtime();
  const uint32_t lane = threadIdx.x;
  const uint32_t t = blockIdx.x * 64u + lane;
  ChunkDesc cd = {nullptr, 0};
  if (t < n) cd = chunks[t];
  const uint32_t nblk = (uint32_t)(cd.len >> 6);
  const uint32_t ntiles = rfl_u32((wave_max_u32(nblk) + (kTB - 1)) / kTB);
  auto swz = [](uint32_t c) -> uint32_t { return (c >> 1) & 7u; };
  const uint32_t slot = lane % kS;
  const uint64_t myptr = reinterpret_cast<uint64_t>(cd.ptr);
  const uint8_t* src[kS];
  uint32_t src_nblk[kS], piece[kS];
#pragma unroll
  for (int i = 0; i < kS; ++i) {
    const int c = i * kCPI + (int)(lane / kS);
    const uint32_t lo = (uint32_t)__shfl((int)(uint32_t)myptr, c, 64);
    const uint32_t hi = (uint32_t)__shfl((int)(uint32_t)(myptr >> 32), c, 64);
    src[i] = reinterpret_cast<const uint8_t*>(((uint64_t)hi << 32) | lo);
    src_nblk[i] = (uint32_t)__shfl((int)nblk, c, 64);
    piece[i] = slot ^ swz((uint32_t)c);
  }
  const uint8_t* dummy = reinterpret_cast<const uint8_t*>(chunks);
  auto issue_tile = [&](uint32_t b, uint32_t tl) {
    if (kMode == 2) return;
#pragma unroll
    for (int i = 0; i < kS; ++i) {
      const uint32_t blk = min(tl * (uint32_t)kTB + (piece[i] >> 2), src_nblk[i] - 1u);
      const uint8_t* g = src_nblk[i] ? src[i] + (uint64_t)blk * 64u + (piece[i] & 3u) * 16u : dummy;
      __builtin_amdgcn_global_load_lds(QS_GP(g), QS_LP(&tile_buf[b][i * kCPI][0]), 16, 0, 0);
    }
  };
  const uint32_t rswz = swz(lane);
  uint32_t st[4] = {kInit0, kInit1, kInit2, kInit3};
  issue_tile(0, 0);
  for (uint32_t tl = 0; tl < ntiles; ++tl) {
    const uint32_t b = tl % kBufs;
    if (tl + 1 < ntiles) {
      issue_tile((tl + 1) % kBufs, tl + 1);
      if (kMode != 2) asm volatile("s_waitcnt vmcnt(8)" ::: "memory");
    } else {
      if (kMode != 2) asm volatile("s_waitcnt vmcnt(0)" ::: "memory");
    }
#pragma unroll
    for (int h = 0; h < kTB; ++h) {
      u32x4 q0 = tile_buf[b][lane][(4 * h + 0) ^ rswz];
      u32x4 q1 = tile_buf[b][lane][(4 * h + 1) ^ rswz];
      u32x4 q2 = tile_buf[b][lane][(4 * h + 2) ^ rswz];
      u32x4 q3 = tile_buf[b][lane][(4 * h + 3) ^ rswz];
      if (tl * (uint32_t)kTB + h < nblk) {
        if (kMode == 1) {
          st[0] ^= q0.x ^ q1.y ^ q2.z ^ q3.w;
          st[1] += q0.y ^ q1.z ^ q2.w ^ q3.x;
          st[2] ^= q0.z + q1.w + q2.x + q3.y;
          st[3] += q0.w + q1.x + q2.y + q3.z;
        } else {
          uint32_t w[16];
          unpack4(w, 0, q0);
          unpack4(w, 1, q1);
          unpack4(w, 2, q2);
          unpack4(w, 3, q3);
          md5_compress(st, w);
        }
      }
    }
    asm volatile("s_waitcnt lgkmcnt(0)" ::: "memory");
  }
  if (t < n) {
    u32x4 o = {st[0], st[1], st[2], st[3]};
    *reinterpret_cast<u32x4*>(digests + 4u * (uint64_t)t) = o;
  }
  const uint64_t m1 = __builtin_amdgcn_s_memtime(), r1 = __builtin_amdgcn_s_memrealtime();
  if (lane == 0) {
    stamps[4 * blockIdx.x + 0] = m0;
    stamps[4 * blockIdx.x + 1] = r0;
    stamps[4 * blockIdx.x + 2] = m1;
    stamps[4 * blockIdx.x + 3] = r1;
  }
}

template <int kMode>
static void run_coal_probe(int B, uint64_t L, uint64_t pad, int reps) {
  uint64_t stride = ((L + 255) & ~uint64_t(255)) + pad;
  uint8_t* d_data;
  CK(hipMalloc(&d_data, stride * (uint64_t)B));
  const uint64_t segs = (L + 1023) / 1024;
  const uint64_t thr = segs * (uint64_t)B;
  hipLaunchKernelGGL(qsmd5_lcg_fill_kernel, dim3((thr + 255) / 256), dim3(256), 0, 0, d_data,
                     stride, L, 12345u, (uint32_t)B, segs);
  std::vector<ChunkDesc> h(B);
  for (int i = 0; i < B; ++i) h[i] = {d_data + stride * (uint64_t)i, L};
  ChunkDesc* d_desc;
  uint32_t* d_dig;
  uint64_t* d_st;
  const int grid = (B + 63) / 64;
  CK(hipMalloc(&d_desc, sizeof(ChunkDesc) * B));
  CK(hipMalloc(&d_dig, 16 * (size_t)B));
  CK(hipMalloc(&d_st, 32 * (size_t)grid));
  CK(hipMemcpy(d_desc, h.data(), sizeof(ChunkDesc) * B, hipMemcpyHostToDevice));
  hipEvent_t e0, e1;
  CK(hipEventCreate(&e0));
  CK(hipEventCreate(&e1));
  std::vector<float> ms(reps);
  for (int r = 0; r < reps; ++r) {
    CK(hipEventRecord(e0, 0));
    hipLaunchKernelGGL(k_coal_probe<kMode>, dim3(grid), dim3(64), 0, 0, d_desc, (uint32_t)B, d_dig, d_st);
    CK(hipEventRecord(e1, 0));
    CK(hipEventSynchronize(e1));
    CK(hipEventElapsedTime(&ms[r], e0, e1));
  }
  std::vector<uint64_t> st(4 * (size_t)grid);
  CK(hipMemcpy(st.data(), d_st, 32 * (size_t)grid, hipMemcpyDeviceToHost));
  std::vector<double> clk, dur;
  for (int g = 0; g < grid; ++g) {
    double dm = (double)(st[4 * g + 2] - st[4 * g]), dr = (double)(st[4 * g + 3] - st[4 * g + 1]);
    if (dr > 0) clk.push_back(dm / dr * 100.0), dur.push_back(dr / 100.0);
  }
  std::sort(clk.begin(), clk.end());
  std::sort(dur.begin(), dur.end());
  std::vector<float> s = ms;
  std::sort(s.begin(), s.end());
  const double med = s[s.size() / 2];
  printf("probe[%s] B=%d L=%llu pad=%llu: median %.3f ms best %.3f ms -> %.1f GB/s; wave clock median %.0f MHz "
         "(p10 %.0f p90 %.0f); wave time median %.1f us max %.1f us\n",
         kMode == 0 ? "full" : kMode == 1 ? "mem-only" : "compute-only", B, (unsigned long long)L,
         (unsigned long long)pad, med, s[0], (double)L * B / (med * 1e-3) / 1e9, clk[clk.size() / 2],
         clk[clk.size() / 10], clk[clk.size() * 9 / 10], dur[dur.size() / 2], dur.back());
  CK(hipFree(d_data));
  CK(hipFree(d_desc));
  CK(hipFree(d_dig));
  CK(hipFree(d_st));
}

int main(int argc, char** argv) {
  const char* mode = argc > 1 ? argv[1] : "all";
  if (!strcmp(mode, "calib")) {
    run_stream_read(4ull << 30, 2);
    run_md5(512, 10485760, 1, false, 1);
    run_md5(131072, 65536, 1, false, 0);
    return 0;
  }
  if (!strcmp(mode, "h2d")) {
    const size_t G = 1ull << 30;
    for (int ns : {1, 2, 4})
      for (size_t piece : {G / 16, 1 * G, 4 * G}) run_h2d(16 * G, piece, ns);
    run_h2d(40 * G, 4 * G, 2);
    for (size_t w : {256ull << 10, 1ull << 20, 10ull << 19})
      for (int ns : {1, 2}) run_h2d_2d(4096, 10 << 20, w, ns);
    for (int ns : {1, 2}) run_h2d(40 * G, 10ull << 20, ns);
    for (int ns : {1, 2}) run_h2d(4 * G, 1ull << 20, ns);
    return 0;
  }
  if (!strcmp(mode, "zc")) {
    g_host_pinned = true;
    run_md5(64, 10485760, 2, true, 1);
    run_md5(512, 10485760, 2, true, 1);
    run_md5(512, 10485760, 2, true, 0);
    run_md5(2048, 10485760, 2, true, 1);
    run_md5(4096, 10485760, 2, true, 1);
    run_md5(4096, 10485760, 2, true, 0);
    return 0;
  }
  if (!strcmp(mode, "coal")) {
    int bad = run_edges(2);
    for (int w : {0, 2}) {
      run_md5(131072, 65536, 5, true, w, 0);
      run_md5(131072, 65536, 5, true, w, 4352);
      run_md5(262144, 32768, 5, true, w, 4352);
      run_md5(65536, 262144, 3, true, w, 4352);
      run_md5(32768, 1 << 20, 3, true, w, 4352);
    }
    return bad ? 1 : 0;
  }
  if (!strcmp(mode, "mem")) {
    run_stream_read(8ull << 30, 5);
    for (int nt = 0; nt < 2; ++nt) {
      run_lane_stream(131072, 65536, 0, nt);
      run_lane_stream(131072, 65536, 4352, nt);
      run_lane_stream(32768, 262144, 4352, nt);
      run_lane_stream(8192, 1 << 20, 4352, nt);
      run_lane_stream(512, 10485760, 0, nt);
    }
    return 0;
  }
  if (!strcmp(mode, "ab")) {
    int bad = run_edges(0) + run_edges(1);
    for (int r = 0; r < 3; ++r) {
      run_md5(512, 10485760, 3, r == 0, 0);
      run_md5(512, 10485760, 3, r == 0, 1);
    }
    run_md5(600, 1 << 20, 3, true, 1);
    run_md5(4096, 1 << 20, 3, true, 1);
    return bad ? 1 : 0;
  }
  if (!strcmp(mode, "issue")) {
    const int iters = 20000;
    printf("  dep v_add_u32      %.2f\n", run_issue(k_dep_add, 64, iters, 64));
    printf("  dep v_add_u32 32 lanes  %.2f\n", run_issue(k_dep_add, 64, iters, 32));
    printf("  dep v_add_u32 16 lanes  %.2f\n", run_issue(k_dep_add, 64, iters, 16));
    printf("  dep v_add_u32 1 lane    %.2f\n", run_issue(k_dep_add, 64, iters, 1));
    printf("  ind v_add_u32 x4 32 lanes %.2f\n", run_issue(k_ind_add, 256, iters, 32));
    printf("  md5 step4 64 lanes %.2f per instr\n", run_issue(k_md5_step4, 256, iters, 64));
    printf("  md5 step4 32 lanes %.2f per instr\n", run_issue(k_md5_step4, 256, iters, 32));
    printf("  md5 step4 1 lane   %.2f per instr\n", run_issue(k_md5_step4, 256, iters, 1));
    printf("  4 v_add + ds_read  %.2f per group\n", run_issue(k_mix_lds, 64, iters, 64));
    return 0;
  }
  if (!strcmp(mode, "stride")) {
    for (uint64_t mib : {10ull, 16ull, 32ull, 64ull}) {
      run_md5(512, mib << 20, 2, false, 1, 0);
      run_md5(512, mib << 20, 2, false, 1, 4096);
      run_md5(512, mib << 20, 2, false, 1, 65536 + 256);
    }
    run_md5(512, 32ull << 20, 2, false, 0, 0);
    run_md5(512, 32ull << 20, 2, false, 0, 4096);
    return 0;
  }
  if (!strcmp(mode, "span")) {
    static const char* names[] = {"in order", "interleaved", "shuffled in 64s", "shuffled all"};
    for (uint64_t pad : {(uint64_t)0, (uint64_t)4352})
      for (int m = 0; m < 4; ++m) {
        g_interleave = m;
        printf("(%s, pad %llu) ", names[m], (unsigned long long)pad);
        run_md5(512, 10ull << 20, 2, false, 1, pad);
      }
    for (uint64_t L : {32ull << 20, 64ull << 20})
      for (uint64_t pad : {(uint64_t)0, (uint64_t)4352})
        for (int m : {0, 2, 3}) {
          g_interleave = m;
          printf("(%s, pad %llu) ", names[m], (unsigned long long)pad);
          run_md5(512, L, 1, false, 1, pad);
        }
    g_interleave = 0;
    return 0;
  }
  if (!strcmp(mode, "fp_pmc")) {
    run_md5(512, 10ull << 20, 1, false, 1, 0);
    run_md5(512, 10ull << 20, 1, false, 1, (54ull << 20) + 4096);
    run_md5(512, 64ull << 20, 1, false, 1, 4096);
    return 0;
  }
  if (!strcmp(mode, "footprint")) {
    for (int rep = 0; rep < 2; ++rep) {
      run_md5(512, 10ull << 20, 2, rep == 0, 1, 0);
      run_md5(512, 10ull << 20, 2, rep == 0, 1, (54ull << 20) + 4096);
      run_md5(512, 10ull << 20, 2, false, 1, (22ull << 20) + 4096);
      run_md5(512, 64ull << 20, 2, false, 1, 4096);
    }
    run_md5(10000, 10ull << 20, 2, true, 1, 0);
    return 0;
  }
  if (!strcmp(mode, "imm")) {
    int bad = run_edges(2) + run_edges(6);
    for (int rep = 0; rep < 2; ++rep)
      for (int w : {2, 6}) {
        run_md5(131072, 65536, 10, rep == 0, w, 4352);
        run_md5(131072, 262144, 6, rep == 0, w, 4352);
      }
    run_md5(100000, 65536 + 17 * 64, 3, true, 6, 4352);
    run_md5(131072, 65536 + 64 * 3, 3, true, 6, 4352);
    return bad ? 1 : 0;
  }
  if (!strcmp(mode, "tlb")) {
    for (uint64_t mib : {32ull, 64ull})
      for (uint64_t pad : {0ull, 4096ull, 1ull << 20, 2ull << 20, (2ull << 20) + 4096, 6ull << 20})
        run_md5(512, mib << 20, 2, false, 1, pad);
    run_md5(512, 10ull << 20, 2, false, 1, 0);
    return 0;
  }
  if (!strcmp(mode, "skew")) {
    int bad = 0;
    for (int w : {1, 3, 4}) {
      bad += run_edges(w);
      for (uint64_t mib : {10ull, 32ull, 64ull}) run_md5(512, mib << 20, 2, mib == 64, w, 0);
      for (uint64_t mib : {32ull, 64ull}) run_md5(512, mib << 20, 2, false, w, 4096);
      run_md5(512, 64ull << 20, 2, false, w, 65536 + 256);
      run_md5(100, (32ull << 20) + 64 * 7 + 13, 2, true, w, 0);
    }
    return bad ? 1 : 0;
  }
  if (!strcmp(mode, "ptrace")) {
    const int B = argc > 2 ? atoi(argv[2]) : 512;
    const uint64_t L = (argc > 3 ? strtoull(argv[3], nullptr, 10) : 64) << 20;
    const uint64_t pad = argc > 4 ? strtoull(argv[4], nullptr, 10) : 4352;
    const uint32_t lanes = argc > 5 ? (uint32_t)atoi(argv[5]) : 64u;
    const uint64_t stride = L + pad;
    uint8_t* d_data;
    CK(hipMalloc(&d_data, stride * (uint64_t)B));
    const uint64_t segs = (L + 1023) / 1024;
    hipLaunchKernelGGL(qsmd5_lcg_fill_kernel, dim3((segs * B + 255) / 256), dim3(256), 0, 0, d_data,
                       stride, L, 12345u, (uint32_t)B, segs);
    std::vector<ChunkDesc> h(B);
    for (int i = 0; i < B; ++i) h[i] = {d_data + (uint64_t)i * stride, L};
    ChunkDesc* d_c;
    uint32_t* d_dig;
    uint64_t* d_tr;
    const int groups = (B + (int)lanes - 1) / (int)lanes;
    CK(hipMalloc(&d_c, sizeof(ChunkDesc) * B));
    CK(hipMalloc(&d_dig, 16 * B));
    CK(hipMalloc(&d_tr, 8 * 1024 * groups));
    CK(hipMemset(d_tr, 0, 8 * 1024 * groups));
    CK(hipMemcpy(d_c, h.data(), sizeof(ChunkDesc) * B, hipMemcpyHostToDevice));
    hipEvent_t e0, e1;
    CK(hipEventCreate(&e0));
    CK(hipEventCreate(&e1));
    CK(hipEventRecord(e0, 0));
    hipLaunchKernelGGL(k_pc_trace, dim3(groups), dim3(128), 0, 0, d_c, nullptr, (uint32_t)B, d_dig,
                       g_skew, d_tr, lanes);
    CK(hipEventRecord(e1, 0));
    CK(hipDeviceSynchronize());
    float ms = 0;
    CK(hipEventElapsedTime(&ms, e0, e1));
    std::vector<uint64_t> tr(1024 * groups);
    CK(hipMemcpy(tr.data(), d_tr, 8 * tr.size(), hipMemcpyDeviceToHost));
    const uint64_t nblk = L / 64;
    printf("ptrace B=%d L=%llu MiB pad=%llu skew=%u lanes=%u: %.2f ms, %.1f cycles/block overall at 2.4 GHz\n",
           B, (unsigned long long)(L >> 20), (unsigned long long)pad, g_skew, lanes, ms,
           ms * 1e-3 * 2.4e9 / (double)nblk);
    {
      double cw = 0, ct = 0, pw = 0, pwr = 0, pt = 0;
      for (int g = 0; g < groups; ++g) {
        const uint64_t* t = &tr[(uint64_t)g * 1024];
        pt += t[1019]; cw += t[1020]; ct += t[1021]; pw += t[1022]; pwr += t[1023];
      }
      const double ph = (double)groups * (double)(nblk / 4);
      printf("  per phase: chain %.0f cycles (%.0f waiting at the barrier); producer %.0f "
             "(%.0f writing the ring incl. load waits, %.0f at the barrier)\n",
             ct / ph, cw / ph, pt / ph, pwr / ph, pw / ph);
    }
    const int pts = (int)std::min<uint64_t>(510, (nblk / 4 + 4095) / 4096);
    for (int g = 0; g < groups; g += std::max(1, groups / 4)) {
      printf("  wg %d: MiB-index:cycles/block@GHz", g);
      for (int k = 1; k < pts; ++k) {
        const uint64_t* a = &tr[(uint64_t)g * 1024 + 2 * (k - 1)];
        const uint64_t* b = &tr[(uint64_t)g * 1024 + 2 * k];
        if (!b[0] || !a[0]) break;
        const double cyc = (double)(b[0] - a[0]), real = (double)(b[1] - a[1]);
        if (k % std::max(1, pts / 16) == 0 || k == pts - 1)
          printf(" %d:%.0f@%.2f", k, cyc / 16384.0, cyc / real * 0.1);
      }
      printf("\n");
    }
    CK(hipFree(d_data));
    CK(hipFree(d_c));
    CK(hipFree(d_dig));
    CK(hipFree(d_tr));
    return 0;
  }
  if (!strcmp(mode, "half5")) {
    int bad = 0;
    bad += run_edges(7);
    for (int rep = 0; rep < 2; ++rep) {
      run_md5(512, 10ull << 20, 5, rep == 0, 1);
      run_md5(512, 10ull << 20, 5, rep == 0, 7);
    }
    return bad ? 1 : 0;
  }
  if (!strcmp(mode, "pace")) {
    int bad = run_edges(1) + run_edges(19);
    for (int rep = 0; rep < 3; ++rep)
      for (int w : {1, 19, 20, 23}) run_md5(512, 10ull << 20, 7, rep == 0, w);
    for (int w : {1, 19, 20}) run_md5(8192, 1ull << 20, 5, true, w);
    return bad ? 1 : 0;
  }
  if (!strcmp(mode, "lead")) {
    int bad = 0;
    for (int w : {30, 31, 32, 33}) bad += run_edges(w);
    for (int rep = 0; rep < 3; ++rep)
      for (int w : {1, 34}) run_md5(512, 10ull << 20, 7, rep == 0, w);
    for (int rep = 0; rep < 4; ++rep)
      for (int w : {1, 30, 31, 32, 33}) run_md5(512, 10ull << 20, 7, rep == 0, w);
    for (int w : {1, 30, 31, 32, 33}) run_md5(8192, 1ull << 20, 5, true, w);
    return bad ? 1 : 0;
  }
  if (!strcmp(mode, "pc2_pace")) {
    for (int rep = 0; rep < 2; ++rep)
      for (int B : {20480, 32768})
        for (int w : {5, 40, 41, 42, 43, 44}) run_md5(B, 1ull << 20, 5, rep == 0, w, 4352);
    return 0;
  }
  if (!strcmp(mode, "lead_pace")) {
    for (int rep = 0; rep < 3; ++rep)
      for (int w : {1, 35, 36, 37, 38, 39}) run_md5(512, 10ull << 20, 7, rep == 0, w);
    for (int w : {1, 37, 38}) run_md5(8192, 1ull << 20, 5, true, w);
    return 0;
  }
  if (!strcmp(mode, "attrib")) {
    int bad = run_edges(1);
    for (int rep = 0; rep < 3; ++rep)
      for (int w : {1, 50, 51, 52}) run_md5(512, 10ull << 20, 5, rep == 0 && w == 1, w);
    return bad ? 1 : 0;
  }
  if (!strcmp(mode, "chaincost")) {
    uint64_t* d_out;
    uint32_t* d_sink;
    CK(hipMalloc(&d_out, 8));
    CK(hipMalloc(&d_sink, 4 * 128));
    const int phases = 4096;
    auto one = [&](auto kern, const char* what) {
      hipLaunchKernelGGL(kern, dim3(1), dim3(128), 0, 0, d_out, d_sink, 16);
      hipLaunchKernelGGL(kern, dim3(1), dim3(128), 0, 0, d_out, d_sink, phases);
      CK(hipDeviceSynchronize());
      uint64_t cyc;
      CK(hipMemcpy(&cyc, d_out, 8, hipMemcpyDeviceToHost));
      printf("  %-58s %.1f cycles/block\n", what, (double)cyc / (phases * kPcHalf));
    };
    one(k_chain_cost<2>, "steps from registers (no LDS, no barrier)");
    one(k_chain_cost<0>, "chain_phase: 16 ds_read_b128 + 1 wait per block");
    one(k_chain_cost<1>, "chain_phase + lds_barrier per 4 blocks (2nd wave barriers only)");
    one(k_chain_cost<0, 32>, "chain_phase, 32 active lanes");
    one(k_chain_cost<0, 16>, "chain_phase, 16 active lanes");
    one(k_chain_cost<0, 1>, "chain_phase, 1 active lane");
    one(k_chain_cost<2, 32>, "steps from registers, 32 active lanes");
    one(k_chain_spread<16>, "reads spread: 1 DS read per 16 VALU");
    one(k_chain_cost<0, 64, 4>, "chain_phase, graded wait on block 0 (lead 4 steps)");
    one(k_chain_cost<0, 64, 8>, "chain_phase, graded wait on block 0 (lead 8 steps)");
    one(k_chain_cost<0, 64, 16>, "chain_phase, graded wait on block 0 (lead 16 steps)");
    one(k_chain_cost<0, 64, 32>, "chain_phase, graded wait on block 0 (lead 32 steps)");
    one(k_chain_cost<1, 64, 16>, "+ lds_barrier per 4 blocks, lead 16");
    u32x4* d_ring;
    CK(hipMalloc(&d_ring, 64 * 16384));
    {
      std::vector<uint32_t> h(64 * 4096);
      for (size_t i = 0; i < h.size(); ++i) h[i] = (uint32_t)i * 2654435761u;
      CK(hipMemcpy(d_ring, h.data(), h.size() * 4, hipMemcpyHostToDevice));
    }
    const int nb = phases * kPcHalf;
    auto ring_one = [&](auto kern, const char* what) {
      hipLaunchKernelGGL(kern, dim3(1), dim3(128), 0, 0, d_out, d_sink, 64, d_ring);
      hipLaunchKernelGGL(kern, dim3(1), dim3(128), 0, 0, d_out, d_sink, nb, d_ring);
      CK(hipDeviceSynchronize());
      uint64_t cyc;
      CK(hipMemcpy(&cyc, d_out, 8, hipMemcpyDeviceToHost));
      printf("  %-58s %.1f cycles/block\n", what, (double)cyc / nb);
    };
    ring_one(k_chain_ring<0>, "continuous LDS ring (no phases, no barrier)");
    ring_one(k_chain_at<0>, "continuous LDS, next reads after step 0");
    ring_one(k_chain_at<4>, "continuous LDS, next reads after step 4");
    ring_one(k_chain_at<8>, "continuous LDS, next reads after step 8");
    ring_one(k_chain_at<16>, "continuous LDS, next reads after step 16");
    ring_one(k_chain_at<32>, "continuous LDS, next reads after step 32");
    ring_one(k_chain_ring<1, 2>, "global ring 2 blocks, default policy");
    ring_one(k_chain_ring<1, 8>, "global ring 8 blocks, default policy");
    ring_one(k_chain_ring<2, 8>, "global ring 8 blocks, sc0 (L2)");
    ring_one(k_chain_ring<2, 64>, "global ring 64 blocks, sc0 (L2)");
    ring_one(k_chain_ring<3, 64>, "global ring 64 blocks, nt");
    ring_one(k_chain_l1<2, 64, false>, "L1 ring 2 slots x 64 lanes (32 KiB)");
    ring_one(k_chain_l1<2, 64, true>, "L1 ring 2 slots x 64 lanes, barrier per block");
    ring_one(k_chain_l1<3, 32, false, false>, "L1 ring 3 slots x 32 live lanes, 1 KiB rows");
    ring_one(k_chain_l1<3, 32, false>, "L1 ring 3 slots x 32 live lanes (24 KiB)");
    ring_one(k_chain_l1<3, 32, true>, "L1 ring 3 slots x 32 live lanes, barrier per block");
    ring_one(k_chain_l1<4, 32, true>, "L1 ring 4 slots x 32 live lanes (32 KiB), barrier");
    ring_one(k_chain_l1<2, 32, true>, "L1 ring 2 slots x 32 live lanes (16 KiB), barrier");
    ring_one(k_chain_l1<5, 16, true>, "L1 ring 5 slots x 16 live lanes (20 KiB), barrier");
    ring_one(k_chain_l1<8, 16, true>, "L1 ring 8 slots x 16 live lanes (32 KiB), barrier");
    ring_one(k_chain_l1<4, 16, true>, "L1 ring 4 slots x 16 live lanes (16 KiB), barrier");
    ring_one(k_chain_l1<2, 16, true>, "L1 ring 2 slots x 16 live lanes (8 KiB), barrier");
    ring_one(k_chain_l1<1, 64, false>, "L1 ring 1 slot x 64 lanes (16 KiB)");
    {
      uint64_t* d_o2;
      CK(hipMalloc(&d_o2, 16));
      auto hand = [&](auto kern, const char* what) {
        hipLaunchKernelGGL(kern, dim3(1), dim3(128), 0, 0, d_o2, d_sink, 64, d_ring);
        hipLaunchKernelGGL(kern, dim3(1), dim3(128), 0, 0, d_o2, d_sink, nb, d_ring);
        CK(hipDeviceSynchronize());
        uint64_t r[2];
        CK(hipMemcpy(r, d_o2, 16, hipMemcpyDeviceToHost));
        printf("  %-58s %.1f cycles/block, %llu stale operand groups\n", what, (double)r[0] / nb,
               (unsigned long long)r[1]);
      };
      hand(k_l1_handoff<0>, "hand-off: 2 slots, producer stores, default policy");
      hand(k_l1_handoff<1>, "hand-off: 2 slots, producer stores sc0");
      hand(k_l1_handoff<2>, "hand-off: 2 slots, producer stores nt");
      CK(hipFree(d_o2));
    }
    CK(hipFree(d_ring));
    CK(hipFree(d_out));
    CK(hipFree(d_sink));
    return 0;
  }
  if (!strcmp(mode, "cross")) {
    int bad = run_edges(5);
    for (int B : {512, 8192, 16384, 20480, 24576, 32768, 49152})
      for (int w : {1, 5, 2}) run_md5(B, 1 << 20, 3, w == 5, w, 4352);
    run_md5(512, 10 << 20, 3, true, 5, 0);
    return bad ? 1 : 0;
  }
  if (!strcmp(mode, "coalfast")) {
    int bad = run_edges(2);
    for (int rep = 0; rep < 2; ++rep) {
      run_coal_probe<0>(131072, 65536, 4352, 5);
      run_md5(131072, 65536, 5, rep == 0, 2, 4352);
    }
    run_coal_probe<0>(65536, 262144, 4352, 3);
    run_md5(65536, 262144, 3, true, 2, 4352);
    run_coal_probe<0>(32768, 1 << 20, 4352, 3);
    run_md5(32768, 1 << 20, 3, true, 2, 4352);
    run_md5(131072, 65536 + 64 * 3, 3, true, 2, 4352);
    run_md5(100000, 65536 + 17 * 64, 3, true, 2, 4352);
    return bad ? 1 : 0;
  }
  if (!strcmp(mode, "probe")) {
    for (int rep = 0; rep < 2; ++rep) {
      run_coal_probe<0>(131072, 65536, 4352, 5);
      run_coal_probe<1>(131072, 65536, 4352, 5);
      run_coal_probe<2>(131072, 65536, 4352, 5);
    }
    run_coal_probe<0>(65536, 262144, 4352, 3);
    run_coal_probe<1>(65536, 262144, 4352, 3);
    run_coal_probe<2>(65536, 262144, 4352, 3);
    run_coal_probe<0>(262144, 65536, 4352, 3);
    run_coal_probe<1>(262144, 65536, 4352, 3);
    run_coal_probe<2>(262144, 65536, 4352, 3);
    run_coal_probe<0>(8192, 1 << 20, 4352, 3);
    return 0;
  }
  if (!strcmp(mode, "prio")) {
    run_stamps(131072, 64 << 10, 20, 4352, 0, 0);
    for (int round = 0; round < 2; ++round)
      for (int prio : {0, 2, 4})
        for (uint64_t kib : {64, 256}) run_stamps(131072, kib << 10, 5, 4352, 0, prio);
    return 0;
  }
  if (!strcmp(mode, "stamps")) {
    for (uint32_t extra : {0u, 4096u})
      for (uint64_t kib : {64, 256}) run_stamps(131072, kib << 10, 6, 4352, extra);
    return 0;
  }
  if (!strcmp(mode, "sat")) {
    run_stream_read(8ull << 30, 5);
    run_md5(131072, 65536, 5, true, 0, 0);
    run_md5(131072, 65536, 5, true, 0, 4352);
    run_md5(262144, 32768, 5, true, 0, 4352);
    run_md5(524288, 16384, 5, true, 0, 4352);
    run_md5(65536, 262144, 3, true, 0, 4352);
    run_md5(16384, 1 << 20, 3, true, 1, 4352);
    run_md5(512, 10485760, 3, true, 0, 0);
    return 0;
  }
  int dev = 0;
  hipDeviceProp_t prop;
  CK(hipGetDeviceProperties(&prop, dev));
  printf("device %s %s CUs=%d clock=%d kHz\n", prop.name, prop.gcnArchName,
         prop.multiProcessorCount, prop.clockRate);
  const int iters = 20000;
  printf("issue (cycles/instr, s_memtime ticks, 1 wave):\n");
  printf("  dep v_add_u32      %.2f\n", run_issue(k_dep_add, 64, iters, 64));
  printf("  ind v_add_u32 x4   %.2f\n", run_issue(k_ind_add, 256, iters, 64));
  printf("  dep v_alignbit     %.2f\n", run_issue(k_dep_alignbit, 64, iters, 64));
  printf("  dep v_bitop3       %.2f\n", run_issue(k_dep_bitop3, 64, iters, 64));
  printf("  dep v_add3_u32     %.2f\n", run_issue(k_dep_add3, 64, iters, 64));
  printf("  md5 step (5 ins)   %.2f per instr\n", run_issue(k_md5_step, 320, iters, 64));
  printf("  md5 step4 (4 ins)  %.2f per instr\n", run_issue(k_md5_step4, 256, iters, 64));
  printf("  4 v_add + ds_read  %.2f per group\n", run_issue(k_mix_lds, 64, iters, 64));
  printf("  dep v_add_u32 2 waves/WG   %.2f\n", run_issue(k_dep_add, 64, iters, 128));
  printf("  dep v_add_u32 8 waves/WG   %.2f\n", run_issue(k_dep_add, 64, iters, 512));
  printf("  dep v_add_u32 16 waves/WG  %.2f\n", run_issue(k_dep_add, 64, iters, 1024));
  int bad = run_edges(0) + run_edges(1);
  const uint64_t L = 10485760;
  for (int w = 0; w < 2; ++w) {
    run_md5(1, L, 3, true, w);
    run_md5(512, L, 5, true, w);
    run_md5(4096, L, 3, true, w);
    run_md5(65536, 65536, 5, true, w);
  }
  run_md5(512, 1 << 20, 5, true, 1);
  run_md5(4096, 1 << 20, 5, true, 1);
  run_md5(262144, 16384, 5, true, 0);
  return bad ? 1 : 0;
}
```

Measured before the change: 61.72 GiB/s.

## Add scalar-fed producer/consumer MD5 kernel feeding message words through SGPRs

Adds a new kernel in which one producer wave loads message blocks, precomputes word+K sums and writes them to a small per-workgroup global ring. Consumer waves, one chain per wave, read them back with s_load_dwordx16 into SGPRs, so the MD5 step arithmetic uses scalar operands instead of LDS or vector loads. A hand-written asm loop double-buffers these scalar loads across the compression steps. The host dispatch picks this path via an env var and a chunk-count threshold, and allocates ring slabs for it. The cost is an extra global write and read round-trip per block, plus barrier synchronisation between producer and consumers.

```diff
diff --git a/qsfs-fuse_amd/csrc/md5_core.h b/qsfs-fuse_amd/csrc/md5_core.h
--- a/qsfs-fuse_amd/csrc/md5_core.h
+++ b/qsfs-fuse_amd/csrc/md5_core.h
@@ -81,6 +81,21 @@
   }
 }
 
+typedef uint32_t u32x16 __attribute__((ext_vector_type(16)));
+template <int I, int kEnd, int kBase>
+__device__ __forceinline__ void md5_steps_mk(uint32_t (&v)[4], const u32x16 (&m)[2]) {
+  if constexpr (I < kEnd) {
+    static_assert(I >= kBase && kEnd <= kBase + 32, "m covers 32 steps from kBase");
+    constexpr int ia = (4 - (I & 3)) & 3;
+    constexpr int ib = (ia + 1) & 3;
+    constexpr int ic = (ia + 2) & 3;
+    constexpr int id = (ia + 3) & 3;
+    const uint32_t t = v[ia] + md5_round_fn<I>(v[ib], v[ic], v[id]) + m[(I - kBase) >> 4][(I - kBase) & 15];
+    v[ia] = v[ib] + __builtin_rotateleft32(t, md5_shift(I));
+    md5_steps_mk<I + 1, kEnd, kBase>(v, m);
+  }
+}
+
 __device__ __forceinline__ void md5_compress_mk(uint32_t (&st)[4], const uint32_t (&mk)[64]) {
   uint32_t v[4] = {st[0], st[1], st[2], st[3]};
   md5_steps_mk<0>(v, mk);
diff --git a/qsfs-fuse_amd/csrc/md5_kernels.hip b/qsfs-fuse_amd/csrc/md5_kernels.hip
--- a/qsfs-fuse_amd/csrc/md5_kernels.hip
+++ b/qsfs-fuse_amd/csrc/md5_kernels.hip
@@ -537,6 +537,319 @@
   pc_body<true, 1, 2>(segs, order, n, digests, col_off, col_w, states, 0u);
 }
 
+constexpr int kSfChains = 3;
+constexpr int kSfHalf = 3;
+constexpr int kSfLanes = 4;
+constexpr uint32_t kSfRecord = 256;
+constexpr uint32_t kSfHalfBytes = 1024;
+constexpr uint32_t kSfRingBytes = 2 * kSfHalfBytes;
+constexpr uint32_t kSfThreads = (kSfChains + 1) * 64;
+
+template <int kOff>
+__device__ __forceinline__ void sf_fetch(u32x16 (&m)[2], const uint8_t* rec) {
+  asm volatile(
+      "s_load_dwordx16 %0, %2, %3 glc\n\t"
+      "s_load_dwordx16 %1, %2, %4 glc\n\t"
+      "s_waitcnt lgkmcnt(0)"
+      : "=&s"(m[0]), "=&s"(m[1])
+      : "s"(rec), "n"(kOff), "n"(kOff + 64)
+      : "memory");
+}
+
+__device__ __forceinline__ void sf_chain_ragged(uint32_t (&st)[4], const uint8_t* cur,
+                                                uint32_t blk0, uint32_t nblk) {
+  for (uint32_t h = 0; h < (uint32_t)kSfHalf; ++h) {
+    if (blk0 + h < nblk) {
+      u32x16 m[2];
+      uint32_t v[4] = {st[0], st[1], st[2], st[3]};
+      sf_fetch<0>(m, cur + h * kSfRecord);
+      md5_steps_mk<0, 32, 0>(v, m);
+      sf_fetch<128>(m, cur + h * kSfRecord);
+      md5_steps_mk<32, 64, 32>(v, m);
+      st[0] += v[0];
+      st[1] += v[1];
+      st[2] += v[2];
+      st[3] += v[3];
+    }
+  }
+  asm volatile("s_barrier" ::: "memory");
+}
+
+#define SF_STEP(AI, AO, B, C, D, MK, ROTR, IMM)                \
+  "v_bitop3_b32 %[t], " B ", " C ", " D " bitop3:" IMM "\n\t"  \
+  "v_add3_u32 %[t], " AI ", " MK ", %[t]\n\t"                  \
+  "v_alignbit_b32 %[t], %[t], %[t], " ROTR "\n\t"              \
+  "v_add_u32_e32 " AO ", %[t], " B "\n\t"
+#define SF_S0 "%[s0]"
+#define SF_S1 "%[s1]"
+#define SF_S2 "%[s2]"
+#define SF_S3 "%[s3]"
+#define SF_V0 "%[v0]"
+#define SF_V1 "%[v1]"
+#define SF_V2 "%[v2]"
+#define SF_V3 "%[v3]"
+#define SF_R4(M0, M1, M2, M3, R0, R1, R2, R3, IMM)              \
+  SF_STEP(SF_V0, SF_V0, SF_V1, SF_V2, SF_V3, M0, R0, IMM)       \
+  SF_STEP(SF_V3, SF_V3, SF_V0, SF_V1, SF_V2, M1, R1, IMM)       \
+  SF_STEP(SF_V2, SF_V2, SF_V3, SF_V0, SF_V1, M2, R2, IMM)       \
+  SF_STEP(SF_V1, SF_V1, SF_V2, SF_V3, SF_V0, M3, R3, IMM)
+#define SF_F0(M0, M1, M2, M3)                                        \
+  SF_STEP(SF_S0, SF_V0, SF_S1, SF_S2, SF_S3, M0, "25", "0xca")       \
+  SF_STEP(SF_S3, SF_V3, SF_V0, SF_S1, SF_S2, M1, "20", "0xca")       \
+  SF_STEP(SF_S2, SF_V2, SF_V3, SF_V0, SF_S1, M2, "15", "0xca")       \
+  SF_STEP(SF_S1, SF_V1, SF_V2, SF_V3, SF_V0, M3, "10", "0xca")
+#define SF_F(M0, M1, M2, M3) SF_R4(M0, M1, M2, M3, "25", "20", "15", "10", "0xca")
+#define SF_G(M0, M1, M2, M3) SF_R4(M0, M1, M2, M3, "27", "23", "18", "12", "0xe4")
+#define SF_H(M0, M1, M2, M3) SF_R4(M0, M1, M2, M3, "28", "21", "16", "9", "0x96")
+#define SF_I(M0, M1, M2, M3) SF_R4(M0, M1, M2, M3, "26", "22", "17", "11", "0x39")
+#define SF_FF                                 \
+  "v_add_u32_e32 %[s0], %[s0], %[v0]\n\t"     \
+  "v_add_u32_e32 %[s1], %[s1], %[v1]\n\t"     \
+  "v_add_u32_e32 %[s2], %[s2], %[v2]\n\t"     \
+  "v_add_u32_e32 %[s3], %[s3], %[v3]\n\t"
+#define SF_LOAD_X(O0, O1, O2)                             \
+  "s_load_dwordx16 s[4:19], vcc, " O0 " glc\n\t"   \
+  "s_load_dwordx16 s[20:35], vcc, " O1 " glc\n\t"  \
+  "s_load_dwordx16 s[36:51], vcc, " O2 " glc\n\t"
+#define SF_LOAD_Y(O0, O1, O2)                             \
+  "s_load_dwordx16 s[52:67], vcc, " O0 " glc\n\t"  \
+  "s_load_dwordx16 s[68:83], vcc, " O1 " glc\n\t"  \
+  "s_load_dwordx16 s[84:99], vcc, " O2 " glc\n\t"
+#define SF_WAIT "s_waitcnt lgkmcnt(0)\n\t"
+__device__ __forceinline__ void sf_chain_whole(uint32_t (&st)[4], const uint8_t* half,
+                                               uint32_t nphases) {
+  static_assert(kSfHalf == 3 && kSfRecord == 256 && kSfHalfBytes == 0x400, "offsets below");
+  uint32_t v0, v1, v2, v3, t;
+  asm volatile(
+      "s_mov_b32 s2, %[n]\n\t"
+      "s_mov_b64 vcc, %[half]\n\t"
+      SF_LOAD_X("0x0", "0x40", "0x80") SF_WAIT
+      "1:\n\t"
+      SF_LOAD_Y("0xc0", "0x100", "0x140")
+      SF_F0("s4", "s5", "s6", "s7") SF_F("s8", "s9", "s10", "s11")
+      SF_F("s12", "s13", "s14", "s15") SF_F("s16", "s17", "s18", "s19")
+      SF_G("s20", "s21", "s22", "s23") SF_G("s24", "s25", "s26", "s27")
+      SF_G("s28", "s29", "s30", "s31") SF_G("s32", "s33", "s34", "s35")
+      SF_H("s36", "s37", "s38", "s39") SF_H("s40", "s41", "s42", "s43")
+      SF_H("s44", "s45", "s46", "s47") SF_H("s48", "s49", "s50", "s51")
+      SF_WAIT SF_LOAD_X("0x180", "0x1c0", "0x200")
+      SF_I("s52", "s53", "s54", "s55") SF_I("s56", "s57", "s58", "s59")
+      SF_I("s60", "s61", "s62", "s63") SF_I("s64", "s65", "s66", "s67") SF_FF
+      SF_F0("s68", "s69", "s70", "s71") SF_F("s72", "s73", "s74", "s75")
+      SF_F("s76", "s77", "s78", "s79") SF_F("s80", "s81", "s82", "s83")
+      SF_G("s84", "s85", "s86", "s87") SF_G("s88", "s89", "s90", "s91")
+      SF_G("s92", "s93", "s94", "s95") SF_G("s96", "s97", "s98", "s99")
+      SF_WAIT SF_LOAD_Y("0x240", "0x280", "0x2c0")
+      SF_H("s4", "s5", "s6", "s7") SF_H("s8", "s9", "s10", "s11")
+      SF_H("s12", "s13", "s14", "s15") SF_H("s16", "s17", "s18", "s19")
+      SF_I("s20", "s21", "s22", "s23") SF_I("s24", "s25", "s26", "s27")
+      SF_I("s28", "s29", "s30", "s31") SF_I("s32", "s33", "s34", "s35") SF_FF
+      SF_F0("s36", "s37", "s38", "s39") SF_F("s40", "s41", "s42", "s43")
+      SF_F("s44", "s45", "s46", "s47") SF_F("s48", "s49", "s50", "s51")
+      SF_WAIT
+      "s_barrier\n\t"
+      "s_xor_b32 vcc_lo, vcc_lo, 0x400\n\t"
+      SF_LOAD_X("0x0", "0x40", "0x80")
+      SF_G("s52", "s53", "s54", "s55") SF_G("s56", "s57", "s58", "s59")
+      SF_G("s60", "s61", "s62", "s63") SF_G("s64", "s65", "s66", "s67")
+      SF_H("s68", "s69", "s70", "s71") SF_H("s72", "s73", "s74", "s75")
+      SF_H("s76", "s77", "s78", "s79") SF_H("s80", "s81", "s82", "s83")
+      SF_I("s84", "s85", "s86", "s87") SF_I("s88", "s89", "s90", "s91")
+      SF_I("s92", "s93", "s94", "s95") SF_I("s96", "s97", "s98", "s99") SF_FF
+      SF_WAIT
+      "s_add_i32 s2, s2, -1\n\t"
+      "s_cmp_lg_u32 s2, 0\n\t"
+      "s_cbranch_scc1 1b"
+      : [s0] "+v"(st[0]), [s1] "+v"(st[1]), [s2] "+v"(st[2]), [s3] "+v"(st[3]),
+        [v0] "=&v"(v0), [v1] "=&v"(v1), [v2] "=&v"(v2), [v3] "=&v"(v3), [t] "=&v"(t)
+      : [n] "s"(nphases), [half] "s"(half)
+      : "memory", "scc", "s2", "s4", "s5", "s6", "s7", "s8", "s9", "s10", "s11", "s12", "s13",
+        "s14", "s15", "s16", "s17", "s18", "s19", "s20", "s21", "s22", "s23", "s24", "s25", "s26",
+        "s27", "s28", "s29", "s30", "s31", "s32", "s33", "s34", "s35", "s36", "s37", "s38", "s39",
+        "s40", "s41", "s42", "s43", "s44", "s45", "s46", "s47", "s48", "s49", "s50", "s51", "s52",
+        "s53", "s54", "s55", "s56", "s57", "s58", "s59", "s60", "s61", "s62", "s63", "s64", "s65",
+        "s66", "s67", "s68", "s69", "s70", "s71", "s72", "s73", "s74", "s75", "s76", "s77", "s78",
+        "s79", "s80", "s81", "s82", "s83", "s84", "s85", "s86", "s87", "s88", "s89", "s90", "s91",
+        "s92", "s93", "s94", "s95", "s96", "s97", "s98", "s99", "vcc");
+}
+#undef SF_WAIT
+#undef SF_LOAD_Y
+#undef SF_LOAD_X
+#undef SF_FF
+#undef SF_I
+#undef SF_H
+#undef SF_G
+#undef SF_F
+#undef SF_F0
+#undef SF_R4
+#undef SF_V3
+#undef SF_V2
+#undef SF_V1
+#undef SF_V0
+#undef SF_S3
+#undef SF_S2
+#undef SF_S1
+#undef SF_S0
+#undef SF_STEP
+
+constexpr int kSfStageRow = 17;
+__device__ __forceinline__ void sf_stage_mk(u32x4 (*stage)[kSfStageRow], uint32_t lane,
+                                            const PcBlockRegs& r, uint32_t off) {
+  uint32_t d[17] = {r.q[0].x, r.q[0].y, r.q[0].z, r.q[0].w, r.q[1].x, r.q[1].y,
+                    r.q[1].z, r.q[1].w, r.q[2].x, r.q[2].y, r.q[2].z, r.q[2].w,
+                    r.q[3].x, r.q[3].y, r.q[3].z, r.q[3].w, r.e};
+  uint32_t w[16];
+#pragma unroll
+  for (int k = 0; k < 16; ++k) w[k] = __builtin_amdgcn_alignbyte(d[k + 1], d[k], off);
+#pragma unroll
+  for (int g = 0; g < 16; ++g) {
+    u32x4 m;
+    m.x = w[md5_word(4 * g + 0)] + Md5Tables::K[4 * g + 0];
+    m.y = w[md5_word(4 * g + 1)] + Md5Tables::K[4 * g + 1];
+    m.z = w[md5_word(4 * g + 2)] + Md5Tables::K[4 * g + 2];
+    m.w = w[md5_word(4 * g + 3)] + Md5Tables::K[4 * g + 3];
+    stage[lane][g] = m;
+  }
+}
+
+template <int kChains>
+__device__ __forceinline__ void sf_flush(const u32x4 (*stage)[kSfStageRow], uint32_t lane,
+                                         uint8_t* wg_ring, uint32_t half) {
+  static_assert(kSfHalf * kSfRecord <= 64 * 16, "one store instruction per chain");
+  asm volatile("s_waitcnt lgkmcnt(0)" ::: "memory");
+  if (lane < kSfHalf * kSfRecord / 16u) {
+#pragma unroll
+    for (int i = 0; i < kChains; ++i) {
+      const u32x4 m = stage[kSfLanes * i + (lane >> 4)][lane & 15u];
+      uint8_t* dst = wg_ring + (uint32_t)i * kSfRingBytes + half * kSfHalfBytes + lane * 16u;
+      *(QS_GLOBAL u32x4*)(reinterpret_cast<uintptr_t>(dst)) = m;
+    }
+  }
+}
+
+template <int kChains, int kDepth, bool kNT, bool kAgentFence, int kProbe = 0>
+__device__ __forceinline__ void sf_body(const ChunkDesc* __restrict__ chunks,
+                                        const uint32_t* __restrict__ order, uint32_t n,
+                                        uint32_t* __restrict__ digests, uint32_t skew,
+                                        uint8_t* ring) {
+  const uint32_t lane = threadIdx.x & 63u;
+  const uint32_t wave = rfl_u32(threadIdx.x >> 6);
+  const bool producer = wave == (uint32_t)kChains;
+  const uint32_t c = lane / (uint32_t)kSfLanes;
+  const uint32_t t = blockIdx.x * (uint32_t)kChains + c;
+  uint32_t idx = 0;
+  ChunkDesc cd = {nullptr, 0};
+  if (c < (uint32_t)kChains && t < n) {
+    idx = order ? order[t] : t;
+    cd = chunks[idx];
+  }
+  uint32_t nblk = (uint32_t)(cd.len >> 6);
+  const bool skewed = skew != 0 && wave_max_u32(nblk) >= kSkewMinBlocks;
+  uint32_t delta = (skewed && nblk) ? skew * ((t * 37u) & 63u) : 0u;
+  const uint32_t phases = rfl_u32((wave_max_u32(nblk + delta) + kSfHalf - 1) / kSfHalf);
+  uint8_t* const wg_ring = ring + (uint64_t)blockIdx.x * (kChains * kSfRingBytes);
+
+  if (producer) {
+    const uint32_t h = lane % (uint32_t)kSfLanes;
+    const bool work = nblk != 0 && h < (uint32_t)kSfHalf;
+    const uintptr_t pa = reinterpret_cast<uintptr_t>(cd.ptr);
+    const uint32_t off = (uint32_t)(pa & 3u);
+    const uint32_t* base = reinterpret_cast<const uint32_t*>(pa & ~uintptr_t(3));
+    const uint32_t last = nblk ? nblk - 1 : 0;
+    __shared__ u32x4 stage[64][kSfStageRow];
+    PcBlockRegs r[kDepth];
+    if constexpr ((kProbe & 2) != 0) {
+#pragma unroll
+      for (int k = 0; k < kDepth; ++k) r[k] = PcBlockRegs{{lane, lane, lane, lane}, lane};
+    }
+    auto load_phase = [&](PcBlockRegs& rs, uint32_t p) {
+      if constexpr ((kProbe & 2) != 0) return;
+      if (work) {
+        const uint32_t j = p * kSfHalf + h;
+        pc_load_block<kNT>(rs, base, off, j < delta ? 0u : min(j - delta, last));
+      }
+    };
+    auto write_phase = [&](const PcBlockRegs& rs, uint32_t p) {
+      if constexpr ((kProbe & 1) == 0) {
+        if (work) sf_stage_mk(stage, lane, rs, off);
+        sf_flush<kChains>(stage, lane, wg_ring, p & 1u);
+      }
+      if constexpr (kAgentFence) __builtin_amdgcn_fence(__ATOMIC_RELEASE, "agent");
+      asm volatile("s_waitcnt vmcnt(0)" ::: "memory");
+    };
+    if (phases > 0) {
+#pragma unroll
+      for (int k = 0; k < kDepth; ++k) load_phase(r[k], (uint32_t)k);
+      write_phase(r[0], 0);
+      load_phase(r[0], kDepth);
+    }
+    asm volatile("s_barrier" ::: "memory");
+    for (uint32_t p0 = 0; p0 < phases; p0 += kDepth) {
+#pragma unroll
+      for (int u = 0; u < kDepth; ++u) {
+        const uint32_t p = p0 + (uint32_t)u;
+        if (p < phases) {
+          if (p + 1 < phases) {
+            write_phase(r[(u + 1) % kDepth], p + 1);
+            load_phase(r[(u + 1) % kDepth], p + 1 + kDepth);
+          }
+          asm volatile("s_barrier" ::: "memory");
+        }
+      }
+    }
+    return;
+  }
+
+  const uint32_t my_t = blockIdx.x * (uint32_t)kChains + wave;
+  const uint32_t src = wave * (uint32_t)kSfLanes;
+  idx = (uint32_t)__builtin_amdgcn_readlane((int)idx, src);
+  nblk = (uint32_t)__builtin_amdgcn_readlane((int)nblk, src);
+  delta = (uint32_t)__builtin_amdgcn_readlane((int)delta, src);
+  const uint32_t ptr_lo = (uint32_t)__builtin_amdgcn_readlane((int)(uint32_t)reinterpret_cast<uintptr_t>(cd.ptr), src);
+  const uint32_t ptr_hi = (uint32_t)__builtin_amdgcn_readlane((int)(uint32_t)(reinterpret_cast<uintptr_t>(cd.ptr) >> 32), src);
+  const uint32_t len_lo = (uint32_t)__builtin_amdgcn_readlane((int)(uint32_t)cd.len, src);
+  const uint32_t len_hi = (uint32_t)__builtin_amdgcn_readlane((int)(uint32_t)(cd.len >> 32), src);
+  const uint8_t* const ptr = reinterpret_cast<const uint8_t*>(((uint64_t)ptr_hi << 32) | ptr_lo);
+  const uint64_t len = ((uint64_t)len_hi << 32) | len_lo;
+  const uint8_t* const my = wg_ring + wave * kSfRingBytes;
+  const uint32_t live_lo = (delta + kSfHalf - 1) / kSfHalf;
+  const uint32_t live_hi = (nblk + delta) / kSfHalf;
+  {
+    uint32_t st[4];
+    asm volatile("v_mov_b32 %0, %1" : "=v"(st[0]) : "s"(kInit0));
+    asm volatile("v_mov_b32 %0, %1" : "=v"(st[1]) : "s"(kInit1));
+    asm volatile("v_mov_b32 %0, %1" : "=v"(st[2]) : "s"(kInit2));
+    asm volatile("v_mov_b32 %0, %1" : "=v"(st[3]) : "s"(kInit3));
+    asm volatile("s_barrier" ::: "memory");
+    uint32_t p = 0;
+    while (p < phases) {
+      const uint8_t* cur = my + (p & 1u) * kSfHalfBytes;
+      if (p >= live_lo && p < live_hi) {
+        sf_chain_whole(st, cur, live_hi - p);
+        p = live_hi;
+      } else {
+        sf_chain_ragged(st, cur, p * kSfHalf - delta, nblk);
+        ++p;
+      }
+    }
+    if (my_t < n) {
+      finish(st, ptr + ((uint64_t)nblk << 6), (uint32_t)(len & 63u), len);
+      u32x4 o = {st[0], st[1], st[2], st[3]};
+      if (lane == 0) *reinterpret_cast<u32x4*>(digests + 4u * (uint64_t)idx) = o;
+    }
+  }
+}
+
+#define QSMD5_SF_KERNEL(NAME, NT, FENCE)                                                      \
+  extern "C" __global__ __launch_bounds__(kSfThreads) void NAME(                              \
+      const ChunkDesc* __restrict__ chunks, const uint32_t* __restrict__ order, uint32_t n,   \
+      uint32_t* __restrict__ digests, uint32_t skew, uint8_t* ring) {                         \
+    sf_body<kSfChains, kPcDepth, NT, FENCE>(chunks, order, n, digests, skew, ring);                      \
+  }
+QSMD5_SF_KERNEL(qsmd5_batch_sf_kernel, false, false)
+QSMD5_SF_KERNEL(qsmd5_batch_sf_nt_kernel, true, false)
+#undef QSMD5_SF_KERNEL
+
 #define QS_GP(p) ((const __attribute__((address_space(1))) void*)(uintptr_t)(p))
 #define QS_LP(p) ((__attribute__((address_space(3))) void*)(uintptr_t)(uint32_t)(uintptr_t)(p))
 
@@ -725,9 +1038,84 @@
 
 #include "md5_launch.h"
 
+#include <stdlib.h>
+#include <string.h>
+
+#include <mutex>
+
 namespace qsmd5 {
 
 static inline void clear_stale_error() { (void)hipGetLastError(); }
+
+static bool scalar_feed_for(uint32_t n) {
+  const char* e = getenv("QSMD5_PC_FEED");
+  if (e && !strcmp(e, "lds")) return false;
+  if (n > kScalarFedMaxChunks) return false;
+  if (e && !strcmp(e, "sgpr")) return true;
+  return kScalarFedDefault;
+}
+
+struct SfSlab {
+  void* raw = nullptr;
+  uint8_t* ring = nullptr;
+  hipEvent_t done = nullptr;
+  int device = -1;
+  bool taken = false;
+};
+constexpr int kSfMaxSlabs = 32;
+static std::mutex g_sf_mu;
+static SfSlab g_sf_slabs[kSfMaxSlabs];
+
+static SfSlab* sf_acquire(hipStream_t s) {
+  hipStreamCaptureStatus cap = hipStreamCaptureStatusNone;
+  if (hipStreamIsCapturing(s, &cap) != hipSuccess || cap != hipStreamCaptureStatusNone) {
+    clear_stale_error();
+    return nullptr;
+  }
+  int dev = -1;
+  if (hipGetDevice(&dev) != hipSuccess) {
+    clear_stale_error();
+    return nullptr;
+  }
+  std::lock_guard<std::mutex> lk(g_sf_mu);
+  SfSlab* fresh = nullptr;
+  for (SfSlab& b : g_sf_slabs) {
+    if (!b.raw) {
+      if (!fresh) fresh = &b;
+      continue;
+    }
+    if (b.taken || b.device != dev) continue;
+    if (hipEventQuery(b.done) == hipSuccess) {
+      b.taken = true;
+      return &b;
+    }
+    clear_stale_error();
+  }
+  if (!fresh) return nullptr;
+  constexpr size_t kChainsMax = (kScalarFedMaxChunks + kSfChains - 1) / kSfChains * kSfChains;
+  void* raw = nullptr;
+  hipEvent_t ev = nullptr;
+  if (hipMalloc(&raw, (kChainsMax + 1) * kSfRingBytes) != hipSuccess ||
+      hipEventCreateWithFlags(&ev, hipEventDisableTiming) != hipSuccess) {
+    if (raw) (void)hipFree(raw);
+    clear_stale_error();
+    return nullptr;
+  }
+  fresh->raw = raw;
+  fresh->ring = reinterpret_cast<uint8_t*>((reinterpret_cast<uintptr_t>(raw) + kSfRingBytes - 1) &
+                                           ~uintptr_t(kSfRingBytes - 1));
+  fresh->done = ev;
+  fresh->device = dev;
+  fresh->taken = true;
+  return fresh;
+}
+
+static void sf_release(SfSlab* slab, hipStream_t s) {
+  const bool ok = hipEventRecord(slab->done, s) == hipSuccess;
+  if (!ok) clear_stale_error();
+  std::lock_guard<std::mutex> lk(g_sf_mu);
+  slab->taken = !ok;
+}
 
 hipError_t launch_batch(const void* chunks, const uint32_t* order, uint32_t n, uint32_t* digests,
                         int kind, hipStream_t s, uint32_t skew_blocks, bool load_nt, uint32_t lanes) {
@@ -739,6 +1127,16 @@
   if (kind == kKernelLatency) {
     const ChunkDesc* c = static_cast<const ChunkDesc*>(chunks);
     const uint32_t skew = skew_blocks / kPcHalf * kPcHalf;
+    if (lanes == 64 && scalar_feed_for(n)) {
+      if (SfSlab* slab = sf_acquire(s)) {
+        hipLaunchKernelGGL(load_nt ? qsmd5_batch_sf_nt_kernel : qsmd5_batch_sf_kernel,
+                           dim3((n + kSfChains - 1) / kSfChains), dim3(kSfThreads), 0, s, c, order, n,
+                           digests, skew, slab->ring);
+        const hipError_t e = hipGetLastError();
+        sf_release(slab, s);
+        return e;
+      }
+    }
     if (lanes == 64)
       hipLaunchKernelGGL(load_nt ? qsmd5_batch_pc64_nt_kernel : qsmd5_batch_pc64_kernel,
                          dim3(pc_groups), dim3(128), 0, s, c, order, n, digests, skew);
diff --git a/qsfs-fuse_amd/csrc/md5_launch.h b/qsfs-fuse_amd/csrc/md5_launch.h
--- a/qsfs-fuse_amd/csrc/md5_launch.h
+++ b/qsfs-fuse_amd/csrc/md5_launch.h
@@ -15,6 +15,9 @@
 constexpr uint32_t kLatencyKernelResident = 256u * 64u;
 constexpr uint32_t kLatency2KernelResident = 2u * 256u * 64u;
 
+constexpr uint32_t kScalarFedMaxChunks = 512;
+constexpr bool kScalarFedDefault = true;
+
 constexpr uint32_t kPcSkewBlocks = 4;
 
 hipError_t launch_batch(const void* chunks, const uint32_t* order, uint32_t n, uint32_t* digests,
diff --git a/ubench/ubench_md5.hip b/ubench/ubench_md5.hip
--- a/ubench/ubench_md5.hip
+++ b/ubench/ubench_md5.hip
@@ -51,6 +51,177 @@
                                                   uint32_t* __restrict__ d, uint32_t skew) {
   pc_body<false, kPcDepth, kPcHalf, false, false, kPcPace, 0, kPcLead, 0, kProbe>(
       c, o, n, d, 0, ~0ull, nullptr, skew, nullptr, 64u);
+}
+
+template <bool kFence>
+__global__ __launch_bounds__(kSfThreads) void k_sf(const ChunkDesc* __restrict__ c,
+                                                   const uint32_t* __restrict__ o, uint32_t n,
+                                                   uint32_t* __restrict__ d, uint32_t skew,
+                                                   uint8_t* ring) {
+  sf_body<kSfChains, kPcDepth, false, kFence>(c, o, n, d, skew, ring);
+}
+template <int kProbe>
+__global__ __launch_bounds__(kSfThreads) void k_sf_attrib(const ChunkDesc* __restrict__ c,
+                                                          const uint32_t* __restrict__ o, uint32_t n,
+                                                          uint32_t* __restrict__ d, uint32_t skew,
+                                                          uint8_t* ring) {
+  sf_body<kSfChains, kPcDepth, false, false, kProbe>(c, o, n, d, skew, ring);
+}
+template <int kC, int kProbe = 0>
+__global__ __launch_bounds__((kC + 1) * 64) void k_sfc(const ChunkDesc* __restrict__ c,
+                                                       const uint32_t* __restrict__ o, uint32_t n,
+                                                       uint32_t* __restrict__ d, uint32_t skew,
+                                                       uint8_t* ring) {
+  sf_body<kC, kPcDepth, false, false, kProbe>(c, o, n, d, skew, ring);
+}
+
+__device__ __forceinline__ uint32_t sf_probe_word(uint32_t p, uint32_t c, uint32_t i) {
+  return (p + 1u) * 0x9E3779B1u + c * 4096u + i;
+}
+template <bool kFence>
+__global__ __launch_bounds__(kSfThreads) void k_sf_probe(uint8_t* ring, uint32_t laps,
+                                                         uint32_t* out) {
+  const uint32_t lane = threadIdx.x & 63u;
+  const uint32_t wave = rfl_u32(threadIdx.x >> 6);
+  if (wave == (uint32_t)kSfChains) {
+    const uint32_t c = lane / kSfLanes, h = lane % kSfLanes;
+    auto write = [&](uint32_t p) {
+      if (c >= (uint32_t)kSfChains || h >= (uint32_t)kSfHalf) return;
+      QS_GLOBAL u32x4* rec = (QS_GLOBAL u32x4*)(reinterpret_cast<uintptr_t>(
+          ring + c * kSfRingBytes + (p & 1u) * kSfHalfBytes + h * kSfRecord));
+      for (uint32_t g = 0; g < 16; ++g) {
+        const uint32_t i = h * 64u + g * 4u;
+        rec[g] = u32x4{sf_probe_word(p, c, i), sf_probe_word(p, c, i + 1),
+                       sf_probe_word(p, c, i + 2), sf_probe_word(p, c, i + 3)};
+      }
+      if constexpr (kFence) __builtin_amdgcn_fence(__ATOMIC_RELEASE, "agent");
+      asm volatile("s_waitcnt vmcnt(0)" ::: "memory");
+    };
+    write(0);
+    asm volatile("s_barrier" ::: "memory");
+    for (uint32_t p = 0; p < laps; ++p) {
+      if (p + 1 < laps) write(p + 1);
+      asm volatile("s_barrier" ::: "memory");
+    }
+    return;
+  }
+  uint32_t bad = 0;
+  asm volatile("s_barrier" ::: "memory");
+  for (uint32_t p = 0; p < laps; ++p) {
+    const uint8_t* half = ring + wave * kSfRingBytes + (p & 1u) * kSfHalfBytes;
+    for (uint32_t h = 0; h < (uint32_t)kSfHalf; ++h) {
+      u32x16 m[2];
+      sf_fetch<0>(m, half + h * kSfRecord);
+      for (int k = 0; k < 32; ++k) bad += m[k >> 4][k & 15] != sf_probe_word(p, wave, h * 64u + k);
+      sf_fetch<128>(m, half + h * kSfRecord);
+      for (int k = 0; k < 32; ++k)
+        bad += m[k >> 4][k & 15] != sf_probe_word(p, wave, h * 64u + 32u + k);
+    }
+    asm volatile("s_barrier" ::: "memory");
+  }
+  if (lane == 0) out[wave] = bad;
+}
+
+template <bool kGlc>
+__global__ __launch_bounds__(576) void k_sload(const uint8_t* base, uint32_t iters, uint64_t* out) {
+  const uint32_t wave = rfl_u32(threadIdx.x >> 6);
+  const uint32_t gw = blockIdx.x * (blockDim.x >> 6) + wave;
+  const uint8_t* p = base + (uint64_t)gw * (kGlc ? 256u : 256u * iters);
+  const uint64_t t0 = __builtin_amdgcn_s_memtime();
+  if constexpr (kGlc)
+    asm volatile(
+        "s_mov_b32 s33, %[n]\n\t"
+        "s_mov_b64 s[34:35], %[p]\n\t"
+        "1:\n\t"
+        "s_load_dwordx16 s[36:51], s[34:35], 0x0 glc\n\t"
+        "s_load_dwordx16 s[52:67], s[34:35], 0x40 glc\n\t"
+        "s_load_dwordx16 s[68:83], s[34:35], 0x80 glc\n\t"
+        "s_load_dwordx16 s[84:99], s[34:35], 0xc0 glc\n\t"
+        "s_waitcnt lgkmcnt(0)\n\t"
+        "s_add_i32 s33, s33, -1\n\t"
+        "s_cmp_lg_u32 s33, 0\n\t"
+        "s_cbranch_scc1 1b"
+        :
+        : [n] "s"(iters), [p] "s"(p)
+        : "memory", "scc", "s33", "s34", "s35", "s36", "s37", "s38", "s39", "s40", "s41", "s42",
+          "s43", "s44", "s45", "s46", "s47", "s48", "s49", "s50", "s51", "s52", "s53", "s54",
+          "s55", "s56", "s57", "s58", "s59", "s60", "s61", "s62", "s63", "s64", "s65", "s66",
+          "s67", "s68", "s69", "s70", "s71", "s72", "s73", "s74", "s75", "s76", "s77", "s78",
+          "s79", "s80", "s81", "s82", "s83", "s84", "s85", "s86", "s87", "s88", "s89", "s90",
+          "s91", "s92", "s93", "s94", "s95", "s96", "s97", "s98", "s99");
+  else
+    asm volatile(
+        "s_mov_b32 s33, %[n]\n\t"
+        "s_mov_b64 s[34:35], %[p]\n\t"
+        "1:\n\t"
+        "s_load_dwordx16 s[36:51], s[34:35], 0x0\n\t"
+        "s_load_dwordx16 s[52:67], s[34:35], 0x40\n\t"
+        "s_load_dwordx16 s[68:83], s[34:35], 0x80\n\t"
+        "s_load_dwordx16 s[84:99], s[34:35], 0xc0\n\t"
+        "s_waitcnt lgkmcnt(0)\n\t"
+        "s_add_u32 s34, s34, 0x100\n\t"
+        "s_addc_u32 s35, s35, 0\n\t"
+        "s_add_i32 s33, s33, -1\n\t"
+        "s_cmp_lg_u32 s33, 0\n\t"
+        "s_cbranch_scc1 1b"
+        :
+        : [n] "s"(iters), [p] "s"(p)
+        : "memory", "scc", "s33", "s34", "s35", "s36", "s37", "s38", "s39", "s40", "s41", "s42",
+          "s43", "s44", "s45", "s46", "s47", "s48", "s49", "s50", "s51", "s52", "s53", "s54",
+          "s55", "s56", "s57", "s58", "s59", "s60", "s61", "s62", "s63", "s64", "s65", "s66",
+          "s67", "s68", "s69", "s70", "s71", "s72", "s73", "s74", "s75", "s76", "s77", "s78",
+          "s79", "s80", "s81", "s82", "s83", "s84", "s85", "s86", "s87", "s88", "s89", "s90",
+          "s91", "s92", "s93", "s94", "s95", "s96", "s97", "s98", "s99");
+  const uint64_t t1 = __builtin_amdgcn_s_memtime();
+  if ((threadIdx.x & 63u) == 0) out[gw] = t1 - t0;
+}
+
+template <bool kGlc>
+static void run_sload(int groups, int waves, uint32_t iters) {
+  const size_t nw = (size_t)groups * waves;
+  const size_t bytes = nw * 256u * (kGlc ? 1u : iters);
+  uint8_t* d;
+  uint64_t* d_out;
+  CK(hipMalloc(&d, bytes));
+  CK(hipMemset(d, 1, bytes));
+  CK(hipMalloc(&d_out, nw * sizeof(uint64_t)));
+  CK(hipDeviceSynchronize());
+  hipLaunchKernelGGL(k_sload<kGlc>, dim3(groups), dim3(waves * 64), 0, 0, d, iters, d_out);
+  CK(hipGetLastError());
+  CK(hipDeviceSynchronize());
+  std::vector<uint64_t> h(nw);
+  CK(hipMemcpy(h.data(), d_out, nw * sizeof(uint64_t), hipMemcpyDeviceToHost));
+  std::sort(h.begin(), h.end());
+  printf("sload[%s] %d workgroups x %d waves: %.0f cycles (s_memtime) per 4 x dwordx16, median wave; %.0f slowest\n",
+         kGlc ? "glc, one record" : "plain, fresh memory", groups, waves,
+         (double)h[nw / 2] / iters, (double)h[nw - 1] / iters);
+  CK(hipFree(d));
+  CK(hipFree(d_out));
+}
+
+template <bool kFence>
+static int run_sf_probe(uint32_t laps) {
+  uint8_t* raw;
+  uint32_t* d_out;
+  CK(hipMalloc(&raw, (kSfChains + 1) * kSfRingBytes));
+  CK(hipMalloc(&d_out, sizeof(uint32_t) * kSfChains));
+  CK(hipMemset(raw, 0, (kSfChains + 1) * kSfRingBytes));
+  CK(hipMemset(d_out, 0xff, sizeof(uint32_t) * kSfChains));
+  uint8_t* ring = reinterpret_cast<uint8_t*>((reinterpret_cast<uintptr_t>(raw) + kSfRingBytes - 1) &
+                                             ~uintptr_t(kSfRingBytes - 1));
+  hipLaunchKernelGGL(k_sf_probe<kFence>, dim3(1), dim3(kSfThreads), 0, 0, ring, laps, d_out);
+  CK(hipGetLastError());
+  CK(hipDeviceSynchronize());
+  uint32_t h[kSfChains];
+  CK(hipMemcpy(h, d_out, sizeof(h), hipMemcpyDeviceToHost));
+  uint64_t bad = 0;
+  for (int w = 0; w < kSfChains; ++w) bad += h[w];
+  printf("sf_probe[%s] %u laps x %d chains x %u dwords: %llu mismatches\n",
+         kFence ? "release fence (agent) + vmcnt(0)" : "vmcnt(0) alone", laps, kSfChains,
+         kSfHalf * 64u, (unsigned long long)bad);
+  CK(hipFree(raw));
+  CK(hipFree(d_out));
+  return bad ? 1 : 0;
 }
 
 template <int kR, int kHalf = kPcHalf>
@@ -505,6 +676,61 @@
   uint64_t t1 = __builtin_amdgcn_s_memtime();
   if (threadIdx.x == 0) out[0] = t1 - t0;
   sink[threadIdx.x] = a + b + c + d;
+}
+
+template <bool kSgpr>
+__global__ void k_step_feed(uint64_t* out, uint32_t* sink, int iters, uint32_t active) {
+  uint32_t a = threadIdx.x, b = 1, c = 2, d = 3;
+  const uint32_t mk = 7;
+  uint64_t t0 = 0, t1 = 0;
+  if ((threadIdx.x & 63u) < active) {
+    t0 = __builtin_amdgcn_s_memtime();
+    for (int i = 0; i < iters; ++i) {
+      if constexpr (kSgpr)
+        asm volatile(REP8(REP8(
+            "v_bitop3_b32 %0, %1, %2, %3 bitop3:0xca\n"
+            "v_add3_u32 %0, %0, %4, %1\n"
+            "v_alignbit_b32 %0, %0, %0, 25\n"
+            "v_add_u32 %0, %0, %1\n"))
+                     : "+v"(a), "+v"(b), "+v"(c), "+v"(d)
+                     : "s"(mk));
+      else
+        asm volatile(REP8(REP8(
+            "v_bitop3_b32 %0, %1, %2, %3 bitop3:0xca\n"
+            "v_add3_u32 %0, %0, %4, %1\n"
+            "v_alignbit_b32 %0, %0, %0, 25\n"
+            "v_add_u32 %0, %0, %1\n"))
+                     : "+v"(a), "+v"(b), "+v"(c), "+v"(d)
+                     : "v"(mk));
+    }
+    t1 = __builtin_amdgcn_s_memtime();
+  }
+  if ((threadIdx.x & 63u) == 0) out[threadIdx.x >> 6] = t1 - t0;
+  sink[threadIdx.x] = a + b + c + d;
+}
+
+template <bool kSgpr>
+static void run_step_feed(int waves, uint32_t active, int iters) {
+  uint64_t* d_out;
+  uint32_t* d_sink;
+  CK(hipMalloc(&d_out, 8 * 16));
+  CK(hipMalloc(&d_sink, 4 * 1024));
+  hipLaunchKernelGGL(k_step_feed<kSgpr>, dim3(1), dim3(waves * 64), 0, 0, d_out, d_sink, 10, active);
+  CK(hipDeviceSynchronize());
+  hipLaunchKernelGGL(k_step_feed<kSgpr>, dim3(1), dim3(waves * 64), 0, 0, d_out, d_sink, iters, active);
+  CK(hipDeviceSynchronize());
+  uint64_t h[16];
+  CK(hipMemcpy(h, d_out, 8 * waves, hipMemcpyDeviceToHost));
+  uint64_t lo = h[0], hi = h[0];
+  for (int w = 1; w < waves; ++w) {
+    lo = std::min(lo, h[w]);
+    hi = std::max(hi, h[w]);
+  }
+  printf("  md5 step4, mk in %s, %2u lanes live, %d waves/WG: %.2f .. %.2f cycles per instr (fastest .. slowest wave)\n",
+         kSgpr ? "SGPR" : "VGPR", active, waves, (double)lo / ((double)iters * 256),
+         (double)hi / ((double)iters * 256));
+  CK(hipFree(d_out));
+  CK(hipFree(d_sink));
 }
 
 __global__ void k_mix_lds(uint64_t* out, uint32_t* sink, int iters) {
@@ -719,8 +945,40 @@
   CK(hipEventCreate(&e0));
   CK(hipEventCreate(&e1));
   const int grid = (B + 63) / 64;
+  const int sf_chains = which == 62 ? 8 : which == 66 ? 1 : which == 67 ? 2 : which == 68 ? 4 : kSfChains;
+  const int sf_grid = (B + sf_chains - 1) / sf_chains;
+  uint8_t* d_ring_raw = nullptr;
+  uint8_t* d_ring = nullptr;
+  if (which >= 60 && which <= 70) {
+    CK(hipMalloc(&d_ring_raw, ((size_t)sf_grid * sf_chains + 1) * kSfRingBytes));
+    d_ring = reinterpret_cast<uint8_t*>((reinterpret_cast<uintptr_t>(d_ring_raw) + kSfRingBytes - 1) &
+                                        ~uintptr_t(kSfRingBytes - 1));
+  }
   auto launch = [&]() {
-    if (which == 0)
+    if (which == 60)
+      hipLaunchKernelGGL(qsmd5_batch_sf_kernel, dim3(sf_grid), dim3(kSfThreads), 0, 0, d_desc,
+                         nullptr, (uint32_t)B, d_dig, g_skew, d_ring);
+    else if (which == 61)
+      hipLaunchKernelGGL(k_sf<true>, dim3(sf_grid), dim3(kSfThreads), 0, 0, d_desc, nullptr,
+                         (uint32_t)B, d_dig, g_skew, d_ring);
+    else if (which >= 63 && which <= 65)
+      hipLaunchKernelGGL(which == 63 ? k_sf_attrib<1> : which == 64 ? k_sf_attrib<2> : k_sf_attrib<3>,
+                         dim3(sf_grid), dim3(kSfThreads), 0, 0, d_desc, nullptr, (uint32_t)B, d_dig,
+                         g_skew, d_ring);
+    else if (which == 62)
+      hipLaunchKernelGGL(k_sfc<8>, dim3(sf_grid), dim3(576), 0, 0, d_desc, nullptr, (uint32_t)B,
+                         d_dig, g_skew, d_ring);
+    else if (which == 66)
+      hipLaunchKernelGGL(k_sfc<1>, dim3(sf_grid), dim3(128), 0, 0, d_desc, nullptr, (uint32_t)B,
+                         d_dig, g_skew, d_ring);
+    else if (which == 67)
+      hipLaunchKernelGGL(k_sfc<2>, dim3(sf_grid), dim3(192), 0, 0, d_desc, nullptr, (uint32_t)B,
+                         d_dig, g_skew, d_ring);
+    else if (which == 68)
+      hipLaunchKernelGGL(k_sfc<4>, dim3(sf_grid), dim3(320), 0, 0, d_desc, nullptr, (uint32_t)B,
+                         d_dig, g_skew, d_ring);
+
+    else if (which == 0)
       hipLaunchKernelGGL(qsmd5_batch_kernel, dim3(grid), dim3(64), 0, 0, d_desc, nullptr,
                          (uint32_t)B, d_dig);
     else if (which == 1)
@@ -846,7 +1104,7 @@
   if (g_host_pinned) printf("[pinned host, zero-copy] ");
   printf("md5[%s] B=%d L=%llu: median %.3f ms best %.3f ms -> %.2f GiB/s total, r1=%.4f GiB/s/chain, "
          "%.1f cycles/block @2.4GHz\n",
-         which == 0 ? "v1" : which == 1 ? "pc" : which == 2 ? "coal" : which == 3 ? "pc-d2" : which == 5 ? "pc-h2" : which == 6 ? "coal-imm" : which == 19 ? "pc (runtime lanes)" : which == 20 ? "pc-r1 (depth 1, no pause)" : which == 21 ? "pace8" : which == 22 ? "pace10" : which == 23 ? "d2-pace8" : which == 24 ? "d2-pace16" : which == 25 ? "d2-pace24" : which == 26 ? "d2-pace32" : which == 30 ? "lead8" : which == 31 ? "lead8+24" : which == 32 ? "lead4+16" : which == 33 ? "lead8+32" : which == 34 ? "lead0 (no graded wait)" : which == 40 ? "pc2 d1 (64u fixed)" : which == 41 ? "pc2 d2" : which == 42 ? "pc2 d2 pace4" : which == 43 ? "pc2 d2 pace8" : which == 44 ? "pc2 d2 pace2" : which == 35 ? "lead8 pace4" : which == 36 ? "lead8 pace12" : which == 37 ? "lead8 pace8 depth3" : which == 38 ? "lead8 pace16 depth3" : which == 39 ? "lead8 no pause" : which == 50 ? "probe: producer writes no ring" : which == 51 ? "probe: producer loads nothing" : which == 52 ? "probe: producer neither loads nor writes" : "pc-d3", B, (unsigned long long)L, med, best, gib / (med / 1e3), (double)L / (1u << 30) / (med / 1e3),
+         which == 0 ? "v1" : which == 1 ? "pc" : which == 2 ? "coal" : which == 3 ? "pc-d2" : which == 5 ? "pc-h2" : which == 6 ? "coal-imm" : which == 19 ? "pc (runtime lanes)" : which == 20 ? "pc-r1 (depth 1, no pause)" : which == 21 ? "pace8" : which == 22 ? "pace10" : which == 23 ? "d2-pace8" : which == 24 ? "d2-pace16" : which == 25 ? "d2-pace24" : which == 26 ? "d2-pace32" : which == 30 ? "lead8" : which == 31 ? "lead8+24" : which == 32 ? "lead4+16" : which == 33 ? "lead8+32" : which == 34 ? "lead0 (no graded wait)" : which == 40 ? "pc2 d1 (64u fixed)" : which == 41 ? "pc2 d2" : which == 42 ? "pc2 d2 pace4" : which == 43 ? "pc2 d2 pace8" : which == 44 ? "pc2 d2 pace2" : which == 35 ? "lead8 pace4" : which == 36 ? "lead8 pace12" : which == 37 ? "lead8 pace8 depth3" : which == 38 ? "lead8 pace16 depth3" : which == 39 ? "lead8 no pause" : which == 50 ? "probe: producer writes no ring" : which == 51 ? "probe: producer loads nothing" : which == 52 ? "probe: producer neither loads nor writes" : which == 60 ? "sf (scalar-fed)" : which == 61 ? "sf, agent release fence" : which == 62 ? "sf, 8 chains per workgroup" : which == 66 ? "sf, 1 chain per workgroup" : which == 67 ? "sf, 2 chains per workgroup" : which == 68 ? "sf, 4 chains per workgroup" : which == 63 ? "sf probe: producer writes no ring" : which == 64 ? "sf probe: producer loads nothing" : which == 65 ? "sf probe: producer neither loads nor writes" : "pc-d3", B, (unsigned long long)L, med, best, gib / (med / 1e3), (double)L / (1u << 30) / (med / 1e3),
          (med / 1e3) * 2.4e9 / (double)(L / 64));
   if (check) {
     std::vector<uint32_t> dig(4 * (size_t)B);
@@ -876,12 +1134,14 @@
     printf("  check %d chunks: %s\n", ncheck, bad ? "FAIL" : "ok");
   }
   if (g_host_pinned) CK(hipHostFree(d_data)); else CK(hipFree(d_data));
+  if (d_ring_raw) CK(hipFree(d_ring_raw));
   CK(hipFree(d_desc));
   CK(hipFree(d_dig));
 }
 
 static int run_edges(int which) {
-  const uint64_t lens[] = {0, 1, 3, 55, 56, 57, 63, 64, 65, 119, 120, 127, 128, 1000, 4096, 8191, 100003};
+  const uint64_t lens[] = {0, 1, 3, 55, 56, 57, 63, 64, 65, 119, 120, 127, 128, 511, 512, 513, 1000,
+                           1024, 1093, 1600, 4096, 8191, 100003};
   const int nl = sizeof(lens) / sizeof(lens[0]);
   int bad = 0;
   uint8_t* d;
@@ -904,7 +1164,15 @@
   CK(hipMalloc(&dg, 16 * n));
   CK(hipMemcpy(dd, desc.data(), sizeof(ChunkDesc) * n, hipMemcpyHostToDevice));
   CK(hipMemset(dg, 0, 16 * n));
-  if (which == 0)
+  uint8_t* ring_raw = nullptr;
+  if (which == 60) {
+    const size_t chains = (size_t)(n + kSfChains - 1) / kSfChains * kSfChains;
+    CK(hipMalloc(&ring_raw, (chains + 1) * kSfRingBytes));
+    uint8_t* ring = reinterpret_cast<uint8_t*>((reinterpret_cast<uintptr_t>(ring_raw) + kSfRingBytes - 1) &
+                                               ~uintptr_t(kSfRingBytes - 1));
+    hipLaunchKernelGGL(qsmd5_batch_sf_kernel, dim3((n + kSfChains - 1) / kSfChains),
+                       dim3(kSfThreads), 0, 0, dd, nullptr, (uint32_t)n, dg, g_skew, ring);
+  } else if (which == 0)
     hipLaunchKernelGGL(qsmd5_batch_kernel, dim3((n + 63) / 64), dim3(64), 0, 0, dd, nullptr,
                        (uint32_t)n, dg);
   else if (which == 1)
@@ -954,6 +1222,7 @@
     }
   }
   printf("edges[%d]: %d cases, %d bad\n", which, n, bad);
+  if (ring_raw) CK(hipFree(ring_raw));
   CK(hipFree(d));
   CK(hipFree(dd));
   CK(hipFree(dg));
@@ -1641,6 +1910,50 @@
       for (uint64_t kib : {64, 256}) run_stamps(131072, kib << 10, 6, 4352, extra);
     return 0;
   }
+  if (!strcmp(mode, "sf_probe")) {
+    const uint32_t laps = argc > 2 ? (uint32_t)atoi(argv[2]) : 4096u;
+    return run_sf_probe<false>(laps) + run_sf_probe<true>(laps);
+  }
+  if (!strcmp(mode, "step_feed")) {
+    for (int waves : {1, 2, 4, 8})
+      for (uint32_t active : {64u, 1u}) {
+        run_step_feed<false>(waves, active, 4000);
+        run_step_feed<true>(waves, active, 4000);
+      }
+    return 0;
+  }
+  if (!strcmp(mode, "sload")) {
+    for (int waves : {1, 2, 4, 8}) run_sload<true>(1, waves, 4096);
+    run_sload<true>(64, 8, 4096);
+    for (int waves : {1, 2, 4, 8}) run_sload<false>(1, waves, 4096);
+    run_sload<false>(64, 8, 4096);
+    return 0;
+  }
+  if (!strcmp(mode, "sf")) {
+    int bad = run_edges(60);
+    if (bad) return 1;
+    for (int r = 0; r < 3; ++r) {
+      run_md5(512, 10485760, 3, r == 0, 1);
+      run_md5(512, 10485760, 3, r == 0, 60);
+    }
+    run_md5(512, 10485760, 3, true, 61);
+    run_md5(512, 10485760, 3, true, 62);
+    return 0;
+  }
+  if (!strcmp(mode, "sf_attrib")) {
+    for (int w : {60, 63, 64, 65}) run_md5(512, 10485760, 2, false, w);
+    return 0;
+  }
+  if (!strcmp(mode, "sf_chains")) {
+    for (int w : {1, 66, 67, 60, 68, 62}) run_md5(512, 10485760, 2, true, w);
+    run_md5(256, 10485760, 2, true, 66);
+    return 0;
+  }
+  if (!strcmp(mode, "sf_nmax")) {
+    for (int B : {512, 768, 1024, 2048, 4096})
+      for (int w : {1, 60}) run_md5(B, 10485760, 2, B <= 1024, w);
+    return 0;
+  }
   if (!strcmp(mode, "sat")) {
     run_stream_read(8ull << 30, 5);
     run_md5(131072, 65536, 5, true, 0, 0);
```

After: 63.19 GiB/s (median of 6 runs). 2.4% higher.
